# fdaPDE/fdaPDE-core

Measured on AMD Instinct MI355X. Metric: DOF/s assemble+solve, 3D P1 Laplacian; SpMV achieved HBM GB/s vs peak, higher is better.
Workload: dtype f64

## Files before the change

### fdapde-core_amd/capi.py

```python
from __future__ import annotations

import ctypes as C
import os

import numpy as np

_HERE = os.path.dirname(os.path.abspath(__file__))
LIB_PATH = os.environ.get("FDAPDE_HIP_LIB") or os.path.join(_HERE, "lib", "libfdapde_hip.so")

OK, EINVAL, ENOMEM, ENODEVICE, EHIP, ENOTINIT, ENOCONV, EUNSUPPORTED, ERCCL = range(9)
LAPLACIAN, DIFFUSION, ADVECTION, REACTION, DT = range(5)
SOLVER_AUTO, SOLVER_CG, SOLVER_BICGSTAB, SOLVER_CG_SR, SOLVER_CG_FUSED, SOLVER_GMRES, SOLVER_DENSE, SOLVER_PMG, SOLVER_AMG = range(9)
ASSEMBLY_ROWS, ASSEMBLY_ATOMIC, ASSEMBLY_COLOURED, ASSEMBLY_PARTITIONED, ASSEMBLY_WAVE = range(5)
MAT_STIFF, MAT_MASS = 0, 1


class Term(C.Structure):
    _fields_ = [("kind", C.c_int32), ("space_varying", C.c_int32), ("coef", C.c_double), ("cst", C.c_double * 9),
                ("data", C.POINTER(C.c_double))]


class Options(C.Structure):
    _fields_ = [("method", C.c_int32), ("maxit", C.c_int32), ("rtol", C.c_double), ("assembly", C.c_int32),
                ("check_every", C.c_int32), ("time_spmv", C.c_int32)]


class Info(C.Structure):
    _fields_ = [("iters", C.c_int32), ("converged", C.c_int32), ("relres", C.c_double), ("t_assemble_ms", C.c_double),
                ("t_solve_ms", C.c_double), ("t_setup_ms", C.c_double), ("spmv_avg_ms", C.c_double), ("spmv_timed", C.c_int32),
                ("method_used", C.c_int32), ("persistent", C.c_int32), ("gather_avg_ms", C.c_double), ("update_avg_ms", C.c_double),
                ("spmv_mean_ms", C.c_double), ("launch_ms", C.c_double)]


SYMBOLS = [
    "fdapde_abi_version", "fdapde_device_count", "fdapde_ctx_create", "fdapde_ctx_destroy", "fdapde_last_error",
    "fdapde_status_string", "fdapde_mesh_upload", "fdapde_dofs_build", "fdapde_dofs_get", "fdapde_dofs_set_boundary", "fdapde_sizes",
    "fdapde_pattern_get", "fdapde_quadrature_nodes", "fdapde_set_operator", "fdapde_set_forcing", "fdapde_set_dirichlet",
    "fdapde_init", "fdapde_assemble_operator", "fdapde_solver_prepare", "fdapde_solve", "fdapde_matrix_values", "fdapde_lump", "fdapde_force", "fdapde_solution",
    "fdapde_info_get", "fdapde_spmv", "fdapde_bench_spmv", "fdapde_tune", "fdapde_stream", "fdapde_synchronize",
    "fdapde_comm_unique_id", "fdapde_comm_init", "fdapde_halo_setup", "fdapde_solve_parabolic",
    "fdapde_lin_compute", "fdapde_lin_solve", "fdapde_eval_pointwise", "fdapde_cell_integrals", "fdapde_comm_init_callback", "fdapde_comm_set_exchange_callback", "fdapde_halo_setup_peers",
    "fdapde_solver_layout", "fdapde_topology_build", "fdapde_topology_get", "fdapde_comm_allreduce", "fdapde_comm_library", "fdapde_solver_layout_kind", "fdapde_solver_layout_partition", "fdapde_rowdist_setup", "fdapde_ctx_clone", "fdapde_comm_count",
    "fdapde_ctx_create_multi", "fdapde_ctx_devices", "fdapde_partition_build", "fdapde_partition_sizes", "fdapde_partition_get", "fdapde_partition_whole",
    "fdapde_partition_peers",
]
PARTITION_ROWDIST, PARTITION_ELEMENTS = 0, 1

_lib = None


def load() -> C.CDLL:
    global _lib
    if _lib is None:
        if not os.path.exists(LIB_PATH):
            raise ImportError(f"{LIB_PATH} is missing: build it with __graft_entry__.build() or `make -C fdapde-core_amd/csrc`. "
                              "There is no CPU fallback.")
        lib = C.CDLL(LIB_PATH)
        lib.fdapde_last_error.restype = C.c_char_p
        lib.fdapde_status_string.restype = C.c_char_p
        lib.fdapde_stream.restype = C.c_void_p
        lib.fdapde_comm_library.restype = C.c_char_p
        lib.fdapde_ctx_destroy.restype = None
        _lib = lib
    return _lib


class FdapdeError(RuntimeError):
    def __init__(self, status, msg):
        super().__init__(f"[status {status}] {msg}")
        self.status = status


def _dp(a):
    return a.ctypes.data_as(C.POINTER(C.c_double))


def _ip(a):
    return a.ctypes.data_as(C.POINTER(C.c_int32))


def _bp(a):
    return a.ctypes.data_as(C.POINTER(C.c_uint8))


class Operator:

    def __init__(self, terms=None):
        self.terms = list(terms or [])

    def __neg__(self):
        return Operator([(k, -c, cst, d) for (k, c, cst, d) in self.terms])

    def __add__(self, o):
        return Operator(self.terms + o.terms)

    def __sub__(self, o):
        return Operator(self.terms + (-o).terms)

    def __rmul__(self, s):
        return Operator([(k, float(s) * c, cst, d) for (k, c, cst, d) in self.terms])

    @property
    def is_symmetric(self):
        return all(k != ADVECTION for (k, _, _, _) in self.terms)

    def c_terms(self):
        arr = (Term * len(self.terms))()
        keep = []
        for t, (k, c, cst, d) in zip(arr, self.terms):
            t.kind, t.coef, t.space_varying = k, c, 0 if d is None else 1
            if cst is not None:
                for i, v in enumerate(np.asarray(cst, dtype=float).reshape(-1)):
                    t.cst[i] = v
            if d is not None:
                dd = np.ascontiguousarray(d, dtype=float)
                keep.append(dd)
                t.data = _dp(dd)
        return arr, keep


def laplacian():
    return Operator([(LAPLACIAN, 1.0, None, None)])


def diffusion(K):
    return Operator([(DIFFUSION, 1.0, np.asarray(K, dtype=float), None)])


def diffusion_field(Kq):
    return Operator([(DIFFUSION, 1.0, None, np.asarray(Kq, dtype=float))])


def advection(b):
    return Operator([(ADVECTION, 1.0, np.asarray(b, dtype=float), None)])


def advection_field(bq):
    return Operator([(ADVECTION, 1.0, None, np.asarray(bq, dtype=float))])


def reaction(c):
    return Operator([(REACTION, 1.0, np.asarray([c], dtype=float), None)])


def reaction_field(cq):
    return Operator([(REACTION, 1.0, None, np.asarray(cq, dtype=float))])


def dt():
    return Operator([(DT, 1.0, None, None)])


class Context:

    def __init__(self, device=0, devices=None):
        self.lib = load()
        self._ctx = C.c_void_p()
        if devices is not None:
            dv = (C.c_int32 * len(devices))(*[int(d) for d in devices])
            rc = self.lib.fdapde_ctx_create_multi(dv, len(devices), C.byref(self._ctx))
        else:
            rc = self.lib.fdapde_ctx_create(-1 if device is None else int(device), C.byref(self._ctx))
        if rc != OK:
            raise FdapdeError(rc, self.lib.fdapde_status_string(rc).decode())
        self.M = self.N = 0
        self.n_cells = self.n_nodes = 0

    def devices(self):
        n = C.c_int32()
        self._check(self.lib.fdapde_ctx_devices(self._ctx, C.byref(n), None, None, None, None))
        dv = (C.c_int32 * n.value)()
        form, tp, tr = C.c_int32(), C.c_double(), C.c_double()
        self._check(self.lib.fdapde_ctx_devices(self._ctx, C.byref(n), dv, C.byref(form), C.byref(tp), C.byref(tr)))
        return dict(devices=list(dv), form=form.value, t_partition_ms=tp.value, t_rank_setup_ms=tr.value)

    def partition_build(self, world, form=PARTITION_ROWDIST):
        self._check(self.lib.fdapde_partition_build(self._ctx, int(world), int(form)))
        self._part_world = int(world)

    def partition_get(self, rank):
        nn, nc = C.c_int64(), C.c_int64()
        self._check(self.lib.fdapde_partition_sizes(self._ctx, int(rank), C.byref(nn), C.byref(nc)))
        nn, nc = nn.value, nc.value
        nodes = np.zeros(nn * self.N)
        cells = np.zeros((nc, self.M + 1), dtype=np.int32)
        bnd = np.zeros(nn, dtype=np.uint8)
        l2g, cids, own = np.zeros(nn, dtype=np.int64), np.zeros(nc, dtype=np.int64), np.zeros(nn, dtype=np.int32)
        self._check(self.lib.fdapde_partition_get(self._ctx, int(rank), _dp(nodes), _ip(cells), _bp(bnd), l2g.ctypes.data_as(C.POINTER(C.c_int64)),
                                                  cids.ctypes.data_as(C.POINTER(C.c_int64)), _ip(own)))
        return dict(nodes=np.ascontiguousarray(nodes.reshape(self.N, nn).T), cells=cells, boundary=bnd, l2g=l2g, cell_ids=cids, owner=own)

    def partition_whole(self):
        part = np.zeros(self.n_cells, dtype=np.int32)
        own = np.zeros(self.n_nodes, dtype=np.int32)
        mask = np.zeros(self.n_nodes, dtype=np.uint64)
# ... 109 lines not shown
            self._check(self.lib.fdapde_set_forcing(self._ctx, None, 0))
            self._force_cols = 1
            return
        f = np.asarray(f_q, dtype=float)
        ncols = 1 if f.ndim == 1 else f.shape[1]
        self._force_cols = ncols
        flat = np.ascontiguousarray(f.reshape(f.shape[0], ncols).T).reshape(-1)
        self._check(self.lib.fdapde_set_forcing(self._ctx, _dp(flat), ncols))

    def set_dirichlet(self, g):
        if g is None:
            self._check(self.lib.fdapde_set_dirichlet(self._ctx, None))
        else:
            g = np.ascontiguousarray(g, dtype=float).reshape(-1)
            self._check(self.lib.fdapde_set_dirichlet(self._ctx, _dp(g)))

    def init(self, assembly=ASSEMBLY_ROWS):
        opt = Options(method=0, maxit=0, rtol=0.0, assembly=assembly, check_every=0, time_spmv=0)
        self._check(self.lib.fdapde_init(self._ctx, C.byref(opt)))

    def assemble_operator(self, which, op: Operator, assembly=ASSEMBLY_ROWS):
        terms, keep = op.c_terms()
        self._check(self.lib.fdapde_assemble_operator(self._ctx, which, len(op.terms), terms, assembly))

    def solver_prepare(self, with_dirichlet=True):
        self._check(self.lib.fdapde_solver_prepare(self._ctx, 1 if with_dirichlet else 0))

    def solve(self, method=SOLVER_AUTO, rtol=1e-10, maxit=0, check_every=0, raise_on_noconv=True, time_spmv=0):
        opt = Options(method=method, maxit=maxit, rtol=rtol, assembly=0, check_every=check_every, time_spmv=time_spmv)
        info = Info()
        rc = self.lib.fdapde_solve(self._ctx, C.byref(opt), C.byref(info))
        if rc != OK and (raise_on_noconv or rc != ENOCONV):
            self._check(rc)
        return info

    def solve_parabolic(self, times, initial_condition, dirichlet=None, method=SOLVER_AUTO, rtol=1e-10, maxit=0):
        times = np.asarray(times, dtype=float).reshape(-1)
        m, nd = times.size, self.sizes()["n_dofs"]
        u0 = np.ascontiguousarray(initial_condition, dtype=float).reshape(-1)
        g = None if dirichlet is None else np.ascontiguousarray(np.asarray(dirichlet, dtype=float).T).reshape(-1)
        out = np.zeros(nd * m)
        opt = Options(method=method, maxit=maxit, rtol=rtol, assembly=0, check_every=0, time_spmv=0)
        info = Info()
        self._check(self.lib.fdapde_solve_parabolic(self._ctx, C.byref(opt), int(m), C.c_double(times[1] - times[0]), _dp(u0),
                                                    None if g is None else _dp(g), _dp(out), C.byref(info)))
        return np.ascontiguousarray(out.reshape(m, nd).T), info

    def lin_compute(self, which=MAT_STIFF, values=None, symmetric=False):
        v = None if values is None else np.ascontiguousarray(values, dtype=float)
        self._check(self.lib.fdapde_lin_compute(self._ctx, which, None if v is None else _dp(v), 1 if symmetric else 0))

    def lin_solve(self, b, method=SOLVER_AUTO, rtol=1e-10, check_every=0, maxit=0):
        b = np.asarray(b, dtype=float)
        one = b.ndim == 1
        B = b.reshape(b.shape[0], -1)
        flat = np.ascontiguousarray(B.T).reshape(-1)
        out = np.zeros_like(flat)
        opt = Options(method=method, maxit=maxit, rtol=rtol, assembly=0, check_every=check_every, time_spmv=0)
        info = Info()
        self._check(self.lib.fdapde_lin_solve(self._ctx, C.byref(opt), _dp(flat), B.shape[1], _dp(out), C.byref(info)))
        X = np.ascontiguousarray(out.reshape(B.shape[1], B.shape[0]).T)
        return (X[:, 0] if one else X), info

    def eval_pointwise(self, locs):
        import scipy.sparse as sp

        locs = np.asarray(locs, dtype=float)
        if locs.ndim == 1:
            locs = locs.reshape(-1, 1)
        nl, s = locs.shape[0], self.sizes()
        flat = np.ascontiguousarray(locs.T).reshape(-1)
        cells = np.zeros(nl, dtype=np.int32)
        vals = np.zeros((nl, s["n_basis"]))
        self._check(self.lib.fdapde_eval_pointwise(self._ctx, C.c_int64(nl), _dp(flat), _ip(cells), _dp(vals)))
        dofs, _, _ = self.dofs_get()
        ok = cells >= 0
        rows = np.repeat(np.nonzero(ok)[0], s["n_basis"])
        cols = dofs[cells[ok]].reshape(-1)
        psi = sp.csr_matrix((vals[ok].reshape(-1), (rows, cols)), shape=(nl, s["n_dofs"]))
        return psi, np.ones(nl), cells

    def eval_areal(self, incidence):
        import scipy.sparse as sp

        inc = sp.csr_matrix(np.asarray(incidence) == 1, dtype=float)
        s = self.sizes()
        meas = np.zeros(self.n_cells)
        pint = np.zeros((self.n_cells, s["n_basis"]))
        self._check(self.lib.fdapde_cell_integrals(self._ctx, _dp(meas), _dp(pint)))
        dofs, _, _ = self.dofs_get()
        D = inc @ meas
        nb = s["n_basis"]
        cellmat = sp.csr_matrix((pint.reshape(-1), (np.repeat(np.arange(self.n_cells), nb), dofs.reshape(-1))),
                                shape=(self.n_cells, s["n_dofs"]))
        psi = sp.diags(1.0 / D) @ (inc @ cellmat)
        return psi.tocsr(), D

    def info(self):
        info = Info()
        self._check(self.lib.fdapde_info_get(self._ctx, C.byref(info)))
        return info

    def matrix_values(self, which=MAT_STIFF):
        out = np.zeros(self.sizes()["nnz"])
        self._check(self.lib.fdapde_matrix_values(self._ctx, which, _dp(out)))
        return out

    def lump(self, which=MAT_MASS):
        out = np.zeros(self.sizes()["n_dofs"])
        self._check(self.lib.fdapde_lump(self._ctx, which, _dp(out)))
        return out

    def force(self, ncols=None):
        have = getattr(self, "_force_cols", 1)
        if ncols is None:
            ncols = have
        if ncols < have:
            raise ValueError(f"force(): the context holds {have} forcing columns, a buffer for {ncols} was asked for")
        out = np.zeros(self.sizes()["n_dofs"] * ncols)
        self._check(self.lib.fdapde_force(self._ctx, _dp(out)))
        return out

    def solution(self):
        out = np.zeros(self.sizes()["n_dofs"])
        self._check(self.lib.fdapde_solution(self._ctx, _dp(out)))
        return out

    def spmv(self, which, x):
        x = np.ascontiguousarray(x, dtype=float)
        y = np.zeros_like(x)
        self._check(self.lib.fdapde_spmv(self._ctx, which, _dp(x), _dp(y)))
        return y

    def bench_spmv(self, reps=50):
        ms, by = C.c_double(), C.c_double()
        self._check(self.lib.fdapde_bench_spmv(self._ctx, reps, C.byref(ms), C.byref(by)))
        return ms.value, by.value

    def solver_layout(self, with_dirichlet=True):
        ni, nz, by = C.c_int64(), C.c_int64(), C.c_double()
        self._check(self.lib.fdapde_solver_layout(self._ctx, 1 if with_dirichlet else 0, C.byref(ni), C.byref(nz), C.byref(by)))
        return ni.value, nz.value, by.value

    def solver_layout_kind(self, with_dirichlet=True):
        k, sy, g, r = C.c_int32(), C.c_int32(), C.c_int32(), C.c_int32()
        self._check(self.lib.fdapde_solver_layout_kind(self._ctx, 1 if with_dirichlet else 0, C.byref(k), C.byref(sy), C.byref(g), C.byref(r)))
        return dict(kind=k.value, sym=sy.value, workgroups=g.value, rows_per_thread=r.value)

    def solver_layout_partition(self, with_dirichlet=True):
        p = C.c_int32()
        self._check(self.lib.fdapde_solver_layout_partition(self._ctx, 1 if with_dirichlet else 0, C.byref(p)))
        return p.value

    @staticmethod
    def comm_unique_id() -> bytes:
        buf = C.create_string_buffer(128)
        rc = load().fdapde_comm_unique_id(buf)
        if rc != OK:
            raise FdapdeError(rc, "fdapde_comm_unique_id failed (RCCL not loadable?)")
        return buf.raw

    def comm_init(self, world, rank, unique_id: bytes):
        self._check(self.lib.fdapde_comm_init(self._ctx, int(world), int(rank), C.c_char_p(unique_id)))

    def rowdist_setup(self, dof_key, dof_owner):
        k = np.ascontiguousarray(dof_key, dtype=np.int64)
        o = np.ascontiguousarray(dof_owner, dtype=np.int32)
        self._check(self.lib.fdapde_rowdist_setup(self._ctx, k.ctypes.data_as(C.POINTER(C.c_int64)), _ip(o)))

    def comm_allreduce(self, values, op="sum"):
        a = np.ascontiguousarray(np.asarray(values, dtype=float)).copy()
        self._check(self.lib.fdapde_comm_allreduce(self._ctx, _dp(a), int(a.size), 0 if op == "sum" else 1))
        return a

    def comm_count(self):
        n = C.c_int32(0)
        self._check(self.lib.fdapde_comm_count(self._ctx, C.byref(n)))
        return int(n.value)

    @staticmethod
    def comm_library():
        return (load().fdapde_comm_library() or b"").decode()

    def comm_init_callback(self, world, rank, allreduce):
        proto = C.CFUNCTYPE(C.c_int, C.c_void_p, C.POINTER(C.c_double), C.c_int64)

        def _cb(user, ptr, count):
            try:
                allreduce(np.ctypeslib.as_array(ptr, shape=(count,)))
                return 0
            except Exception:
                return 1

        self._ar_cb = proto(_cb)
        self._check(self.lib.fdapde_comm_init_callback(self._ctx, int(world), int(rank), self._ar_cb, None))

    def halo_setup(self, n_if_global, local_dof, if_index, owned):
        local_dof = np.ascontiguousarray(local_dof, dtype=np.int32)
        if_index = np.ascontiguousarray(if_index, dtype=np.int32)
        owned = np.ascontiguousarray(owned, dtype=np.uint8)
        self._check(self.lib.fdapde_halo_setup(self._ctx, C.c_int64(int(n_if_global)), C.c_int64(local_dof.size), _ip(local_dof),
                                               _ip(if_index), _bp(owned)))

    def comm_set_exchange_callback(self, exchange):
        proto = C.CFUNCTYPE(C.c_int, C.c_void_p, C.c_int32, C.POINTER(C.c_int32), C.POINTER(C.c_int64), C.POINTER(C.c_double), C.POINTER(C.c_double))

        def _cb(user, n_peers, ranks, offs, send, recv):
            try:
                off = np.ctypeslib.as_array(offs, shape=(n_peers + 1,))
                n = int(off[-1])
                exchange(np.ctypeslib.as_array(ranks, shape=(n_peers,)), off, np.ctypeslib.as_array(send, shape=(n,)),
                         np.ctypeslib.as_array(recv, shape=(n,)))
                return 0
            except Exception:
                return 1

        self._xchg_cb = proto(_cb)
        self._check(self.lib.fdapde_comm_set_exchange_callback(self._ctx, self._xchg_cb, None))

    def halo_setup_peers(self, peer_rank, peer_off, peer_dof, owned):
        peer_rank = np.ascontiguousarray(peer_rank, dtype=np.int32)
        peer_off = np.ascontiguousarray(peer_off, dtype=np.int64)
        peer_dof = np.ascontiguousarray(peer_dof, dtype=np.int32)
        owned = np.ascontiguousarray(owned, dtype=np.uint8)
        self._check(self.lib.fdapde_halo_setup_peers(self._ctx, C.c_int32(peer_rank.size), _ip(peer_rank),
                                                     peer_off.ctypes.data_as(C.POINTER(C.c_int64)), _ip(peer_dof), _bp(owned)))

    def tune(self, key, value):
        self._check(self.lib.fdapde_tune(self._ctx, key.encode(), int(value)))

    def stream(self):
        return self.lib.fdapde_stream(self._ctx)

    def synchronize(self):
        self._check(self.lib.fdapde_synchronize(self._ctx))
```

### fdapde-core_amd/csrc/capi.hip

```cpp
#include <algorithm>
#include <chrono>
#include <cmath>
#include <cstdio>
#include <cstdlib>
#include <cstring>
#include <new>

#include <dlfcn.h>
#include <hip/hip_ext.h>
#include <rccl/rccl.h>

#include "context.h"
#include "engine.h"

using namespace fdapde_engine;

extern "C" {

int fdapde_abi_version(void) { return FDAPDE_ABI_VERSION; }

int fdapde_device_count(void) {
    int n = 0;
    if (hipGetDeviceCount(&n) != hipSuccess) return 0;
    return n;
// ... 90 lines not shown
        if (c->h_sc) (void)hipHostFree(c->h_sc);
        (void)hipEventDestroy(c->ev0), (void)hipEventDestroy(c->ev1), (void)hipEventDestroy(c->ev_p0), (void)hipEventDestroy(c->ev_p1);
        for (hipEvent_t e : c->ev_spmv) (void)hipEventDestroy(e);
        (void)hipStreamDestroy(c->stream);
    }
    delete c->lin_state;
    delete c;
}

int fdapde_ctx_clone(const fdapde_ctx* src, fdapde_ctx** out) {
    if (!src || !out) return FDAPDE_EINVAL;
    *out = nullptr;
    if (src->group) return fdapde_engine::g_clone(src, out);
    fdapde_ctx* c = nullptr;
    if (int rc = fdapde_ctx_create(src->has_device ? src->device : -1, &c)) return rc;
    const int rc = fdapde_engine::e_ctx_clone(src, c);
    if (rc != FDAPDE_OK) {
        const_cast<fdapde_ctx*>(src)->err = "fdapde_ctx_clone: " + c->err;
        fdapde_ctx_destroy(c);
        return rc;
    }
    *out = c;
    return FDAPDE_OK;
}

const char* fdapde_last_error(const fdapde_ctx* c) { return c ? c->err.c_str() : "null context"; }

int fdapde_mesh_upload(fdapde_ctx* c, int M, int N, int64_t n_nodes, const double* nodes, int64_t n_cells,
                       const int32_t* cells, const uint8_t* bnd) {
    if (!c) return FDAPDE_EINVAL;
    if (c->group && M == 2 && N == 3)
        return fail(c, FDAPDE_EUNSUPPORTED, "fdapde_mesh_upload: a surface mesh (Triangulation<2,3>) takes a one-GPU context; the multi-device partitioner "
                                            "and its ranks are built for planar and volume meshes");
    if (c->group && M == 1)
        return fail(c, FDAPDE_EUNSUPPORTED, "fdapde_mesh_upload: a 1-D mesh (interval or linear network, Triangulation<1,N>) takes a one-GPU context; the "
                                            "multi-device partitioner and its ranks are built for planar and volume meshes");
    c->space_ready = c->dev_ready = c->colour_ready = c->fq_blk_ready = c->fq_bc_ready = c->stiff_stat_valid = false;
    c->assembled[0] = c->assembled[1] = c->force_ready = c->solved = c->dirichlet_applied = false;
    c->op.clear(), c->coef_of_op = false, c->fq_i.clear(), c->fq_cols = 0, c->g_i.clear(), c->have_g = false;
    if (c->topo_ready) dev_topology_release(&c->topo), c->topo_ready = false;
    c->mesh_on_dev = false;
    if (int rc = host_set_mesh(c->hs, M, N, n_nodes, nodes, n_cells, cells, bnd, c->err)) return rc;
    if (c->has_device) {
        const HostSpace& hs = c->hs;
        if (hipSetDevice(c->device) != hipSuccess || c->mesh_nodes.upload(hs.nodes.data(), hs.nodes.size(), c->stream) != hipSuccess ||
            c->mesh_cells.upload(hs.cells.data(), hs.cells.size(), c->stream) != hipSuccess ||
            c->mesh_nbnd.upload(hs.node_bnd.data(), hs.node_bnd.size(), c->stream) != hipSuccess || hipStreamSynchronize(c->stream) != hipSuccess) {
            c->mesh_nodes.release(), c->mesh_cells.release(), c->mesh_nbnd.release();
            c->err = "fdapde_mesh_upload: copying the mesh to the device failed";
            return FDAPDE_EHIP;
        }
        c->mesh_on_dev = true;
    }
    fdapde_engine::partition_free(c);
    if (c->group) fdapde_engine::g_mesh_changed(c);
    return FDAPDE_OK;
}

int fdapde_sizes(const fdapde_ctx* c, int64_t* n_dofs, int64_t* nnz, int32_t* n_basis, int32_t* n_quadrature, int64_t* n_edges) {
    if (!c || !c->space_ready) return FDAPDE_ENOTINIT;
    if (n_dofs) *n_dofs = c->hs.n_dofs;
    if (nnz) *nnz = c->hs.nnz;
    if (n_basis) *n_basis = c->hs.nb;
    if (n_quadrature) *n_quadrature = c->hs.nq;
    if (n_edges) *n_edges = c->hs.n_edges;
    return FDAPDE_OK;
}

int fdapde_dofs_build(fdapde_ctx* c, int order, int64_t* n_dofs) {
    if (!c) return FDAPDE_EINVAL;
    if (c->group) return fdapde_engine::g_dofs_build(c, order, n_dofs);
    return fdapde_engine::e_dofs_build(c, order, n_dofs);
}
int fdapde_topology_build(fdapde_ctx* c, int64_t* n_facets, int64_t* n_edges) {
    if (!c) return FDAPDE_EINVAL;
    return fdapde_engine::e_topology_build(c, n_facets, n_edges);
}
int fdapde_topology_get(fdapde_ctx* c, int32_t* neighbors, int32_t* cell_facets, int32_t* facet_nodes, int32_t* facet_cells, uint8_t* facet_boundary, int32_t* edge_nodes, uint8_t* edge_boundary, int32_t* face_edges) {
    if (!c) return FDAPDE_EINVAL;
    return fdapde_engine::e_topology_get(c, neighbors, cell_facets, facet_nodes, facet_cells, facet_boundary, edge_nodes, edge_boundary, face_edges);
}
int fdapde_dofs_set_boundary(fdapde_ctx* c, const uint8_t* bnd) {
    if (!c) return FDAPDE_EINVAL;
    if (c->group) return fdapde_engine::g_dofs_set_boundary(c, bnd);
    return fdapde_engine::e_dofs_set_boundary(c, bnd);
}
int fdapde_dofs_get(const fdapde_ctx* c, int32_t* dofs, uint8_t* bnd, double* coords) {
    if (!c) return FDAPDE_EINVAL;
    return fdapde_engine::e_dofs_get(c, dofs, bnd, coords);
}
int fdapde_pattern_get(const fdapde_ctx* c, int32_t* rowptr, int32_t* colidx) {
    if (!c) return FDAPDE_EINVAL;
    return fdapde_engine::e_pattern_get(c, rowptr, colidx);
}
int fdapde_quadrature_nodes(fdapde_ctx* c, double* out) {
    if (!c) return FDAPDE_EINVAL;
    return fdapde_engine::e_quadrature_nodes(c, out);
}
int fdapde_set_operator(fdapde_ctx* c, int32_t n_terms, const fdapde_term* terms) {
    if (!c) return FDAPDE_EINVAL;
    if (c->group) return fdapde_engine::g_set_operator(c, n_terms, terms);
    return fdapde_engine::e_set_operator(c, n_terms, terms);
}
int fdapde_set_forcing(fdapde_ctx* c, const double* f_q, int32_t n_cols) {
    if (!c) return FDAPDE_EINVAL;
    if (c->group) return fdapde_engine::g_set_forcing(c, f_q, n_cols);
    return fdapde_engine::e_set_forcing(c, f_q, n_cols);
}
int fdapde_set_dirichlet(fdapde_ctx* c, const double* g) {
    if (!c) return FDAPDE_EINVAL;
    if (c->group) return fdapde_engine::g_set_dirichlet(c, g);
    return fdapde_engine::e_set_dirichlet(c, g);
}
int fdapde_assemble_operator(fdapde_ctx* c, int32_t which, int32_t n_terms, const fdapde_term* terms, int32_t assembly) {
    if (!c) return FDAPDE_EINVAL;
    if (c->group) return fdapde_engine::g_assemble_operator(c, which, n_terms, terms, assembly);
    return fdapde_engine::e_assemble_operator(c, which, n_terms, terms, assembly);
}
int fdapde_init(fdapde_ctx* c, const fdapde_options* opt) {
    if (!c) return FDAPDE_EINVAL;
    if (c->group) return fdapde_engine::g_init(c, opt);
    return fdapde_engine::e_init(c, opt);
}
int fdapde_eval_pointwise(fdapde_ctx* c, int64_t n_locs, const double* locs_colmajor, int32_t* cell_ids, double* values) {
    if (!c) return FDAPDE_EINVAL;
    return fdapde_engine::e_eval_pointwise(c, n_locs, locs_colmajor, cell_ids, values);
}
int fdapde_cell_integrals(fdapde_ctx* c, double* measure, double* psi_int) {
    if (!c) return FDAPDE_EINVAL;
    return fdapde_engine::e_cell_integrals(c, measure, psi_int);
}
int fdapde_solver_prepare(fdapde_ctx* c, int32_t with_dirichlet) {
    if (!c) return FDAPDE_EINVAL;
    if (c->group) return fdapde_engine::g_solver_prepare(c, with_dirichlet);
    return fdapde_engine::e_solver_prepare(c, with_dirichlet);
}
int fdapde_solver_layout(fdapde_ctx* c, int32_t with_dirichlet, int64_t* n_interior, int64_t* nnz_interior, double* streamed_bytes) {
    if (!c) return FDAPDE_EINVAL;
    if (c->group) return fdapde_engine::g_layout_kind(c, with_dirichlet, nullptr, nullptr, nullptr, nullptr);
    return fdapde_engine::e_solver_layout(c, with_dirichlet, n_interior, nnz_interior, streamed_bytes);
}
int fdapde_solver_layout_kind(fdapde_ctx* c, int32_t with_dirichlet, int32_t* kind, int32_t* symmetric_storage, int32_t* workgroups, int32_t* rows_per_thread) {
    if (!c) return FDAPDE_EINVAL;
    if (c->group) return fdapde_engine::g_layout_kind(c, with_dirichlet, kind, symmetric_storage, workgroups, rows_per_thread);
    return fdapde_engine::e_solver_layout_kind(c, with_dirichlet, kind, symmetric_storage, workgroups, rows_per_thread);
}
int fdapde_solver_layout_partition(fdapde_ctx* c, int32_t with_dirichlet, int32_t* partition) {
    int32_t kind = 0;
    if (int rc = fdapde_solver_layout_kind(c, with_dirichlet, &kind, nullptr, nullptr, nullptr)) return rc;
    const fdapde_ctx::Persist& ps = c->ps[with_dirichlet ? 1 : 0];
    if (partition) *partition = (kind == 2 || kind == 3) && ps.ok ? (ps.meta.bisect ? 1 : 0) : -1;
    return FDAPDE_OK;
}
int fdapde_solve(fdapde_ctx* c, const fdapde_options* opt, fdapde_info* info) {
    if (!c) return FDAPDE_EINVAL;
    if (c->group && opt && opt->method == FDAPDE_SOLVER_AMG) return fdapde_engine::fail(c, FDAPDE_EUNSUPPORTED, "FDAPDE_SOLVER_AMG takes one-GPU contexts, not a multi-device context");
    if (c->group) return fdapde_engine::g_solve(c, opt, info);
    return fdapde_engine::e_solve(c, opt, info);
}
int fdapde_solve_parabolic(fdapde_ctx* c, const fdapde_options* opt, int32_t n_times, double delta_t, const double* initial_condition, const double* dirichlet, double* solution, fdapde_info* info) {
    if (!c) return FDAPDE_EINVAL;
    if (c->group && opt && opt->method == FDAPDE_SOLVER_AMG) return fdapde_engine::fail(c, FDAPDE_EUNSUPPORTED, "FDAPDE_SOLVER_AMG takes one-GPU contexts, not a multi-device context");
    if (c->group) return fdapde_engine::g_solve_parabolic(c, opt, n_times, delta_t, initial_condition, dirichlet, solution, info);
    return fdapde_engine::e_solve_parabolic(c, opt, n_times, delta_t, initial_condition, dirichlet, solution, info);
}
int fdapde_lin_compute(fdapde_ctx* c, int32_t which, const double* values, int32_t symmetric) {
    if (!c) return FDAPDE_EINVAL;
    if (c->group) return fdapde_engine::g_lin_compute(c, which, values, symmetric);
    return fdapde_engine::e_lin_compute(c, which, values, symmetric);
}
int fdapde_lin_solve(fdapde_ctx* c, const fdapde_options* opt, const double* b, int32_t n_rhs, double* x, fdapde_info* info) {
    if (!c) return FDAPDE_EINVAL;
    if (c->group && opt && opt->method == FDAPDE_SOLVER_AMG) return fdapde_engine::fail(c, FDAPDE_EUNSUPPORTED, "FDAPDE_SOLVER_AMG takes one-GPU contexts, not a multi-device context");
    if (c->group) return fdapde_engine::g_lin_solve(c, opt, b, n_rhs, x, info);
    return fdapde_engine::e_lin_solve(c, opt, b, n_rhs, x, info);
}
int fdapde_matrix_values(fdapde_ctx* c, int32_t which, double* values) {
    if (!c) return FDAPDE_EINVAL;
    if (c->group) return fdapde_engine::g_matrix_values(c, which, values);
    return fdapde_engine::e_matrix_values(c, which, values);
}
int fdapde_lump(fdapde_ctx* c, int32_t which, double* diag) {
    if (!c) return FDAPDE_EINVAL;
    if (c->group) return fdapde_engine::g_lump(c, which, diag);
    return fdapde_engine::e_lump(c, which, diag);
}
int fdapde_force(fdapde_ctx* c, double* force) {
    if (!c) return FDAPDE_EINVAL;
    if (c->group) return fdapde_engine::g_force(c, force);
    return fdapde_engine::e_force(c, force);
}
int fdapde_solution(fdapde_ctx* c, double* solution) {
    if (!c) return FDAPDE_EINVAL;
    if (c->group) return fdapde_engine::g_solution(c, solution);
    return fdapde_engine::e_solution(c, solution);
}
int fdapde_spmv(fdapde_ctx* c, int32_t which, const double* x, double* y) {
    if (!c) return FDAPDE_EINVAL;
    if (c->group) return fdapde_engine::g_spmv(c, which, x, y);
    return fdapde_engine::e_spmv(c, which, x, y);
}
int fdapde_bench_spmv(fdapde_ctx* c, int32_t reps, double* avg_ms, double* algorithmic_bytes) {
    if (!c) return FDAPDE_EINVAL;
    if (c->group) return fail(c, FDAPDE_EUNSUPPORTED, "fdapde_bench_spmv: a multi-device context wires its own ranks");
    return fdapde_engine::e_bench_spmv(c, reps, avg_ms, algorithmic_bytes);
}
int fdapde_comm_unique_id(void* out128) {
    return fdapde_engine::e_comm_unique_id(out128);
}
int fdapde_comm_init(fdapde_ctx* c, int32_t world, int32_t rank, const void* unique_id128) {
    if (!c) return FDAPDE_EINVAL;
    if (c->group) return fail(c, FDAPDE_EUNSUPPORTED, "fdapde_comm_init: a multi-device context wires its own ranks");
    return fdapde_engine::e_comm_init(c, world, rank, unique_id128);
}
int fdapde_comm_allreduce(fdapde_ctx* c, double* host_inout, int32_t n, int32_t op) {
    if (!c) return FDAPDE_EINVAL;
    if (c->group) return fail(c, FDAPDE_EUNSUPPORTED, "fdapde_comm_allreduce: a multi-device context wires its own ranks");
    return fdapde_engine::e_comm_allreduce(c, host_inout, n, op);
}
int fdapde_comm_count(fdapde_ctx* c, int32_t* ranks) {
    if (!c) return FDAPDE_EINVAL;
    return fdapde_engine::e_comm_count(c, ranks);
}
int fdapde_comm_init_callback(fdapde_ctx* c, int32_t world, int32_t rank, fdapde_allreduce_fn fn, void* user) {
    if (!c) return FDAPDE_EINVAL;
    if (c->group) return fail(c, FDAPDE_EUNSUPPORTED, "fdapde_comm_init_callback: a multi-device context wires its own ranks");
    return fdapde_engine::e_comm_init_callback(c, world, rank, fn, user);
}
int fdapde_halo_setup(fdapde_ctx* c, int64_t n_if_global, int64_t n_if_local, const int32_t* local_dof, const int32_t* if_index, const uint8_t* owned) {
    if (!c) return FDAPDE_EINVAL;
    if (c->group) return fail(c, FDAPDE_EUNSUPPORTED, "fdapde_halo_setup: a multi-device context wires its own ranks");
    return fdapde_engine::e_halo_setup(c, n_if_global, n_if_local, local_dof, if_index, owned);
}
int fdapde_rowdist_setup(fdapde_ctx* c, const int64_t* dof_key, const int32_t* dof_owner) {
    if (!c) return FDAPDE_EINVAL;
    if (c->group) return fail(c, FDAPDE_EUNSUPPORTED, "fdapde_rowdist_setup: a multi-device context wires its own ranks");
    return fdapde_engine::e_rowdist_setup(c, dof_key, dof_owner);
}
int fdapde_comm_set_exchange_callback(fdapde_ctx* c, fdapde_exchange_fn fn, void* user) {
    if (!c) return FDAPDE_EINVAL;
    if (c->group) return fail(c, FDAPDE_EUNSUPPORTED, "fdapde_comm_set_exchange_callback: a multi-device context wires its own ranks");
    return fdapde_engine::e_comm_set_exchange_callback(c, fn, user);
}
int fdapde_halo_setup_peers(fdapde_ctx* c, int32_t n_peers, const int32_t* peer_rank, const int64_t* peer_off, const int32_t* peer_dof, const uint8_t* owned) {
    if (!c) return FDAPDE_EINVAL;
    if (c->group) return fail(c, FDAPDE_EUNSUPPORTED, "fdapde_halo_setup_peers: a multi-device context wires its own ranks");
    return fdapde_engine::e_halo_setup_peers(c, n_peers, peer_rank, peer_off, peer_dof, owned);
}

int fdapde_ctx_create_multi(const int32_t* devices, int32_t n_devices, fdapde_ctx** out) {
    return fdapde_engine::g_create(devices, n_devices, out);
}
int fdapde_ctx_devices(const fdapde_ctx* c, int32_t* n_devices, int32_t* devices, int32_t* form, double* t_partition_ms, double* t_rank_setup_ms) {
    if (!c) return FDAPDE_EINVAL;
    return fdapde_engine::g_info(c, n_devices, devices, form, t_partition_ms, t_rank_setup_ms);
}
int fdapde_partition_build(fdapde_ctx* c, int32_t world, int32_t form) {
    if (!c) return FDAPDE_EINVAL;
    if (c->group) return fail(c, FDAPDE_EUNSUPPORTED, "fdapde_partition_build: a multi-device context partitions its mesh itself (fdapde_dofs_build)");
    return fdapde_engine::e_partition_build(c, world, form);
}
int fdapde_partition_sizes(const fdapde_ctx* c, int32_t rank, int64_t* n_nodes, int64_t* n_cells) {
    if (!c) return FDAPDE_EINVAL;
    return fdapde_engine::e_partition_sizes(c, rank, n_nodes, n_cells);
}
int fdapde_partition_get(fdapde_ctx* c, int32_t rank, double* nodes_colmajor, int32_t* cells, uint8_t* boundary, int64_t* node_ids, int64_t* cell_ids, int32_t* node_owner) {
    if (!c) return FDAPDE_EINVAL;
    return fdapde_engine::e_partition_get(c, rank, nodes_colmajor, cells, boundary, node_ids, cell_ids, node_owner);
}
int fdapde_partition_whole(fdapde_ctx* c, int32_t* cell_rank, int32_t* node_owner, uint64_t* node_ranks) {
    if (!c) return FDAPDE_EINVAL;
    return fdapde_engine::e_partition_whole(c, cell_rank, node_owner, node_ranks);
}
int fdapde_partition_peers(fdapde_ctx* c, int32_t rank, int32_t* n_peers, int32_t* peer_rank, int64_t* peer_off, int32_t* peer_node, uint8_t* owned, int64_t* n_shared) {
    if (!c) return FDAPDE_EINVAL;
    return fdapde_engine::e_partition_peers(c, rank, n_peers, peer_rank, peer_off, peer_node, owned, n_shared);
}

int fdapde_info_get(const fdapde_ctx* c, fdapde_info* info) {
    if (!c || !info) return FDAPDE_EINVAL;
    *info = c->info;
    return FDAPDE_OK;
}

const char* fdapde_comm_library(void) { return g_rccl.path.c_str(); }

int fdapde_tune(fdapde_ctx* c, const char* key, int32_t value) {
    if (!c || !key) return FDAPDE_EINVAL;
    if (!c->dev_ready) return fail(c, FDAPDE_ENOTINIT, "call fdapde_dofs_build first");
    if (c->group) return fdapde_engine::g_tune(c, key, value);
    const std::string k(key);
    drop_graph(c);
    if (k == "spmv_variant" && value >= 0 && value <= 2) c->spmv_variant = value;
    else if (k == "spmv_team" && (value == 2 || value == 4 || value == 8 || value == 16 || value == 32 || value == 64)) {
        if (value != c->spmv_team) c->sp_built[0] = c->sp_built[1] = false, c->sp_cur = -1, c->solved = false, c->scaled_owner = fdapde_ctx::kScaledNone;
        c->spmv_team = value;
    }
    else if (k == "spmv_unroll" && value >= 1 && value <= 8) c->spmv_unroll = value;
    else if (k == "spmv_ablate") c->spmv_ablate = value;
    else if (k == "spmv_c16" && (value == 0 || value == 1)) c->spmv_c16 = value;
    else if (k == "spmv_deep" && (value == 0 || value == 1)) c->spmv_deep = value;
    else if (k == "cgf_split" && (value == 0 || value == 1)) c->cgf_split = value;
    else if (k == "cgf_v" && (value == 1 || value == 2 || value == 4 || value == 8)) c->cgf_v = value;
    else if (k == "use_graph" && (value == 0 || value == 1)) c->use_graph = value;
    else if (k == "cgf_band" && (value == 0 || value == 1)) c->cgf_band = value;
    else if (k == "cgf_nt" && value >= 0 && value <= 15) c->cgf_nt = value;
    else if (k == "cgf_lazy" && (value == 0 || value == 1)) c->cgf_lazy = value;
    else if (k == "multi_rhs" && (value == 0 || value == 1)) c->multi_rhs = value;
    else if (k == "asm_fq_block" && (value == 0 || value == 1)) c->asm_fq_block = value;
    else if (k == "asm_fuse_mass" && value >= 0 && value <= 3) c->asm_fuse_mass = value;
    else if (k == "asm_items" && (value == 0 || value == 1)) c->asm_items = value;
    else if (k == "asm_items_fuse" && (value == 0 || value == 1)) c->asm_items_fuse = value;
    else if (k == "bicg_restart" && (value == 0 || value == 1)) c->bicg_restart = value;
    else if (k == "bicg_shadow" && value >= 0 && value <= 2) c->bicg_shadow = value;
    else if (k == "gmres_m" && value >= 2 && value <= 200) c->gmres_m = value;
    else if (k == "persist_exp_lds" && (value == 0 || value == 1)) {
        c->persist_exp_lds = value;
        c->ps[0].tried = c->ps[0].ok = c->ps[1].tried = c->ps[1].ok = false, c->scaled_owner = fdapde_ctx::kScaledNone;
        fdapde_engine::drop_graph(c);
    }
    else if (k == "dense_rows" && value >= 0 && value <= 8192) c->dense_rows = value, c->lin_dense.ready = false, c->lin_dense.failed = false;
    else if (k == "dense_after" && value >= 0) c->dense_after = value;
    else if (k == "dense_block" && (value == 0 || value == 1)) c->dense_block = value;
    else if (k == "dense_direct" && (value == 0 || value == 1)) c->dense_direct = value;
    else if (k == "dense_fold" && (value == 0 || value == 1)) c->dense_fold = value;
    else if (k == "dense_multi" && (value == 0 || value == 1)) c->dense_multi = value;
    else if (k == "pmg_inner_tol_exp" && value >= 1 && value <= 12) c->pmg_inner_rtol = std::pow(10.0, -(double)value);
    else if (k == "pmg_inner_maxit" && value >= 1) c->pmg_inner_maxit = value;
    else if (k == "pmg_auto" && (value == 0 || value == 1)) c->pmg_auto = value;
    else if (k == "pmg_blocked" && (value == 0 || value == 1)) c->pmg_blocked = value;
    else if (k == "pmg_smooth" && (value == 0 || value == 1)) c->pmg_smooth = value;
    else if (k == "pmg_setup_check" && (value == 0 || value == 1)) c->pmg_setup_check = value;
    else if (k == "amg_coarse_rows" && value >= 1 && value <= 8192) c->amg_coarse_rows = value;
    else if (k == "amg_setup_check" && (value == 0 || value == 1)) c->amg_setup_check = value;
    else if (k == "pmg_restart" && value >= 2 && value <= 50) c->pmg_restart = (int)value;
    else if (k == "pmg_outer" && (value == 0 || value == 1)) c->pmg_outer = value;
    else if (k == "pmg_auto_rows" && value >= 0) c->pmg_auto_rows = value;
    else if (k == "pmg_auto_first_rows" && value >= 0) c->pmg_auto_first_rows = value;
    else if (k == "dense_bulk" && (value == 0 || value == 1)) c->dense_bulk = value;
    else if (k == "dense_hostb" && (value == 0 || value == 1)) c->dense_hostb = value;
    else if (k == "small_rows" && value >= 0) c->small_rows = value;
    else if (k == "small_front_rows" && value >= 0) c->small_front_rows = value;
    else if (k == "auto_gmres" && (value == 0 || value == 1)) c->auto_gmres = value;
    else if (k == "asm_split_varying" && (value == 0 || value == 1)) c->asm_split_varying = value;
    else if (k == "asm_row_stat" && (value == 0 || value == 1)) c->asm_row_stat = value, c->stiff_stat_valid = false;
    else if (k == "asm_fq_bc" && (value == 0 || value == 1)) c->asm_fq_bc = value, c->fq_bc_ready = c->fq_bc_ready && value;
    else if (k == "persist" && (value == 0 || value == 1)) c->persist = value, c->persist_broken = false;
    else if (k == "persist_time" && (value == 0 || value == 1)) c->persist_time = value;
    else if (k == "persist_coop" && (value == 0 || value == 1)) c->persist_coop = value;
    else if (k == "persist_bicg" && (value == 0 || value == 1)) c->persist_bicg = value;
    else if (k == "persist_fill_fused" && (value == 0 || value == 1)) c->persist_fill_fused = value;
    else if (k == "persist_prefetch" && (value == 0 || value == 1)) c->persist_prefetch = value;
    else if (k == "persist_cols" && (value == 0 || value == 1)) c->persist_cols = value;
    else if (k == "persist_direct" && (value == 0 || value == 1)) c->persist_direct = value;
    else if (k == "persist_wide_gj" && (value == 4 || value == 6 || value == 12)) {
        c->persist_wide_gj = value;
        for (auto& ps : c->ps) ps.attr_set = nullptr;
    }
    else if ((k == "persist_wide" && (value == 0 || value == 1)) || (k == "persist_max_wg" && value >= 0)) {
        if (k == "persist_wide") c->persist_wide = value;
        else c->persist_max_wg = value;
        for (auto& ps : c->ps) ps.tried = ps.ok = ps.filled = false;
    }
    else if (k == "persist_direct_spin_us" && value >= 0 && value <= 1000000) c->persist_direct_spin_us = value;
    else if (k == "persist_single_rows" && value >= 0 && value <= 8192) {
        c->persist_single_rows = value;
        for (auto& ps : c->ps) ps.tried = ps.ok = ps.filled = false;
    }
    else if (k == "persist_partition" && value >= 0 && value <= 2) {
        c->persist_partition = value;
        for (auto& ps : c->ps) ps.tried = ps.ok = ps.filled = false;
    }
    else if (k == "persist_late" && (value == 0 || value == 1)) {
        c->persist_late = value;
        for (auto& ps : c->ps) ps.tried = ps.ok = ps.filled = false;
    }
    else if (k == "rowdist_max_wg" && value >= 0) {
        c->rd.max_wg = value;
        for (auto& L : c->rd.lay) L.tried = L.ok = false;
    } else if (k == "rowdist_share" && value >= 1) {
        c->rd.max_wg = std::max(1, c->n_cu / value);
        for (auto& L : c->rd.lay) L.tried = L.ok = false;
    } else if (k == "rowdist_timeout_first_ms" && value >= 1) c->rd.timeout_first_ms = value;
    else if (k == "rowdist_flat_gather" && value >= -1 && value <= 1) c->rd.flat_gather = value;
    else if (k == "persist_timeout_us" && value >= 100 && value <= 10000000) c->persist_timeout_us = value;
    else if (k == "persist_debug_stall" && value >= 0) c->persist_debug_stall = value;
    else if (k == "persist_retry" && value == 1) c->persist_broken = false, c->persist_retry_in = 0, c->persist_backoff = 8;
    else if (k == "blocked" && value >= 0 && value <= 2) c->blocked = value;
    else if (k == "persist_gather_waves" && (value == 1 || value == 4)) c->persist_gather_waves = value;
    else if (k == "persist_poll_sleep" && value >= 0 && value <= 3) c->persist_poll_sleep = value;
    else if (k == "persist_balance" && (value == 0 || value == 1)) {
        c->persist_balance = value;
        for (auto& ps : c->ps) ps.tried = ps.ok = ps.filled = false;
    } else if (k == "persist_sym" && value >= 0 && value <= 2) {
        c->persist_sym = value;
        for (auto& ps : c->ps) ps.tried = ps.ok = ps.filled = false;
    }
    else if (k == "spmv_ntv" && value >= -1 && value <= 1) c->spmv_ntv = value;
    else if (k == "spmv_bpx" && value >= 1 && value <= 1024) {
        c->spmv_grid = 8 * value;
        HIPCHK(c, hipSetDevice(c->device));
        HIPCHK(c, hipStreamSynchronize(c->stream));
        HIPCHK(c, c->part_a.alloc(2 * (size_t)c->spmv_grid));
    } else return fail(c, FDAPDE_EINVAL, "unknown tuning key or value out of range");
    return FDAPDE_OK;
}

void* fdapde_stream(fdapde_ctx* c) { return c ? (void*)c->stream : nullptr; }

int fdapde_synchronize(fdapde_ctx* c) {
    if (!c) return FDAPDE_EINVAL;
    if (int rc = need_device(c)) return rc;
    if (c->group)
        if (int rc = fdapde_engine::g_synchronize(c)) return rc;
    HIPCHK(c, hipSetDevice(c->device));
    HIPCHK(c, hipStreamSynchronize(c->stream));
    HIPCHK(c, hipDeviceSynchronize());
    return FDAPDE_OK;
}

}
```

### fdapde-core_amd/csrc/context.h

```cpp
#ifndef FDAPDE_CONTEXT_H
#define FDAPDE_CONTEXT_H

#include <cstdint>
#include <memory>
#include <functional>
#include <string>
#include <vector>

#include <dlfcn.h>
#include <hip/hip_ext.h>
#include <hip/hip_runtime.h>
#include <rccl/rccl.h>

#include "../../include/fdapde_hip.h"
#include "dev_persist.h"
#include "dev_setup.h"
#include "dev_topology.h"
#include "internal.h"

namespace fdapde_engine {
struct Group;
struct AmgHierarchy;
}
namespace fdapde_hip {
// ... 207 lines not shown
    int persist_direct_spin_us = 2000;
    int32_t* h_ctl = nullptr;
    double* h_sc = nullptr;
    int spmv_grid = 0, rb_per_band = 0, vec_grid = 0, n_rb = 0, cg_grid = 0;
    int spmv_variant = 2;
    int spmv_team = 16, spmv_unroll = 4, spmv_ablate = 0;
    int lds_limit = 96 * 1024;
    DBuf<int32_t> sp_rowptr[2], sp_colidx[2], sp_map[2], sp_tbase[2], sp_vrow[2];
    int64_t sp_nv[2] = {0, 0};
    int sval_layout = -2;
    DBuf<uint16_t> sp_col16[2];
    int64_t sp_wide[2] = {0, 0};
    int spmv_ntv = -1;
    int sp_team = 0;
    int spmv_c16 = 1;
    int use_graph = 0;
    hipGraphExec_t cg_graph_exec = nullptr;
    GraphKey cg_graph_key{};
    int cgf_lazy = 1;
    int cgf_nt = 7;
    int cgf_band = 1;
    int cgf_split = 0;
    int cgf_v = 8;
    int spmv_deep = 0;
    int64_t sp_nnz[2] = {0, 0};
    bool sp_built[2] = {false, false};
    int sp_cur = -1;
    bool sval_stale = false;
    const double* sval_A = nullptr;
    int persist_fill_fused = 0;
    enum { kScaledNone = 0, kScaledSolve, kScaledParabolic, kScaledLin, kScaledPmg };
    int scaled_owner = kScaledNone;
    ncclComm_t comm = nullptr;
    fdapde_allreduce_fn ar_fn = nullptr;
    void* ar_user = nullptr;
    std::vector<double> ar_host;
    DBuf<double> ar_dev;
    int world = 1, rank = 0;
    bool halo_ready = false;
    int64_t n_if = 0, n_loc_if = 0;
    DBuf<int32_t> halo_dof, halo_pos;
    DBuf<int32_t> halo_inv, if_slot;
    DBuf<uint8_t> owned;
    DBuf<double> hbuf, sbuf;
    bool peer_mode = false;
    fdapde_exchange_fn xchg_fn = nullptr;
    void* xchg_user = nullptr;
    std::vector<int32_t> peer_rank;
    std::vector<int64_t> peer_off;
    DBuf<int32_t> peer_send_dof;
    DBuf<int32_t> peer_src_off, peer_src;
    DBuf<double> peer_sendbuf, peer_recvbuf;
    std::vector<double> xchg_send_h, xchg_recv_h;
    struct PeerDirect {
        bool on = false;
        int (*arrive)(void*) = nullptr;
        void* user = nullptr;
        int parity = 0, ar_parity = 0;
        int64_t n_send = 0;
        DBuf<const double*> remote[2];
        DBuf<double> slots;
        DBuf<const double*> slot_ptr;
    } xd;
    static constexpr int kSlotDoubles = 64;
    DBuf<double> lin_mat;
    bool lin_ready = false, lin_symmetric = false;
    DBuf<double> lin_sq;
    bool lin_sq_ready = false;
    int multi_rhs = 1;
    SolveStateHolder* lin_state = nullptr;
    int n_cu = 0;
    int persist = 1;
    int persist_time = 1;
    int persist_balance = 1;
    int persist_sym = 2;
    int persist_gather_waves = 4, persist_poll_sleep = 2;
    bool persist_broken = false;
    int persist_retry_in = 0, persist_backoff = 8;
    struct Persist {
        bool tried = false, ok = false;
        PersistLayout meta;
        int32_t lds_cap = 0, imp_cap = 0;
        size_t lds_bytes = 0;
        DBuf<int32_t> slot_dof, sl_off, ell_src, exp_off, imp_off, imp_pos;
        DBuf<int32_t> ell_col;
        bool stream = false;
        bool exp_lds = false;
        DBuf<int64_t> ell_off;
        DBuf<uint16_t> ell_code, exp_slot;
        DBuf<double> ell_val;
        DBuf<unsigned long long> amax;
        DBuf<uint8_t> wg_late;
        DBuf<unsigned long long> board;
        DBuf<unsigned long long> board_cols;
        int per_cu = 0;
        bool filled = false;
        uint32_t epoch_next = 0;
        const void* attr_set = nullptr;
        bool built_plain = false;
    } ps[2];
    struct RowDist {
        bool ready = false;
        std::vector<int32_t> owner_i;
        std::vector<int64_t> key_i;
        DBuf<uint8_t> owned;
        int max_wg = 0;
        int flat_gather = -1;
        int timeout_first_ms = 2000;
        struct Layout {
            bool tried = false, ok = false;
            Persist ps;
            int32_t n_ghost = 0, G_tot = 0, g_base = 0;
            DBuf<int32_t> rexp_off, rexp_peer, rexp_pos;
            DBuf<uint16_t> rexp_slot;
            DBuf<uint8_t> wg_late;
            DBuf<unsigned long long> rboard;
            DBuf<unsigned long long*> peer_pboard, peer_dboard;
            std::vector<void*> ipc_opened;
            std::vector<int32_t> x_rank;
            std::vector<int64_t> x_soff, x_roff;
            DBuf<int32_t> x_send_dof, x_recv_dof;
            DBuf<double> x_sendbuf, x_recvbuf;
        } lay[2];
    } rd;
    DBuf<double> persist_stats;
    DBuf<double> persist_x;
    DBuf<double> persist_xs;
    int persist_wide_gj = 12;
    int persist_wide = 1;
    int persist_max_wg = 0;
    double persist_launch_ms = 0;
    int persist_host_below = 32768;
    int persist_cols = 1;
    DBuf<double> cols_b, cols_r, cols_x, cols_sc, cols_part;
    DBuf<int32_t> cols_ctl;
    struct EvalGrid {
        bool ready = false;
        DBuf<int32_t> ptr, cells, dims;
        DBuf<double> lo, invh;
        void release() { ptr.release(), cells.release(), dims.release(), lo.release(), invh.release(), ready = false; }
    } eval_grid;
    DBuf<double> eval_locs, eval_vals;
    DBuf<int32_t> eval_out;
    std::function<int()> persist_tail;
    int h_ctl_seen = 4;
    bool ev1_at_end = false;
    int64_t small_rows = 8192;
    int64_t small_front_rows = 2048;
    bool front_used = false;
    bool tail_in_launch = false;
    bool defer_end_sync = false;
    int persist_single_rows = 2048;
    int persist_prefetch = 1;
    int persist_partition = 2;
    int persist_late = 0;
    int persist_plain = 0;
    int persist_bicg = 1;
    int persist_coop = 0;
    int persist_timeout_us = 5000;
    int persist_debug_stall = 0;
    struct Blocked {
        bool tried = false, ok = false, filled = false;
        PersistLayout meta;
        int32_t imp_cap = 0;
        size_t lds_bytes = 0;
        DBuf<int32_t> slot_dof, sl_off, ell_src, imp_off, imp_dof, drop_dof;
        DBuf<int64_t> ell_off;
        DBuf<uint16_t> ell_code;
        DBuf<double> ell_val;
    } bk[2];
    int bk_cur = -1;
    int blocked = 1;
    DevTopology topo;
    bool topo_ready = false;
    bool part_ready = false, wave_ready = false;
    int32_t part_colours = 0;
    int64_t n_parts = 0;
    DBuf<int32_t> part_cells, part_off, part_slots, wave_slots;
    DBuf<uint8_t> part_shared;
    std::vector<double> persist_host_stats;
    struct Pmg {
        fdapde_ctx* coarse = nullptr;
        bool ready = false;
        int64_t init_seen = -1;
        double extra_seen = 0.0;
        DBuf<int32_t> pa, pb;
        DBuf<int32_t> fine_cell;
        DBuf<int32_t> rt_ptr, rt_idx;
        DBuf<double> rt_w, dinv, vec, part, dots, basis;
        int np = 1;
        double setup_ms = 0;
        int last_coarse_iters = 0, last_coarse_calls = 0;
        DBuf<int32_t> flag;
        const double* fine_A = nullptr;
        int64_t fine_key = -1;
        int fine_bnd = -1;
        double omega = 0.0;
        const double* omega_A = nullptr;
        int64_t omega_key = -1;
        int omega_bnd = -1;
        double omega_extra = 0.0;
        SolveState coarse_ss;
    } pmg;
    fdapde_engine::AmgHierarchy* amg = nullptr;
    fdapde_engine::AmgHierarchy* amg_lin = nullptr;
    int64_t amg_lin_epoch = 0;
    int64_t amg_coarse_rows = 1024;
    int amg_setup_check = 0;
    int64_t init_count = 0;
    bool matrix_dirty = true;
    bool last_init_rows = false;
    double pmg_inner_rtol = 1e-1;
    int pmg_inner_maxit = 200;
    int pmg_auto = 1;
    int pmg_outer = 0;
    int pmg_setup_check = 0;
    int pmg_restart = 50;
    int pmg_smooth = 1;
    int64_t pmg_auto_first_rows = 1000000;
    int64_t open_solves = 0;
    int pmg_blocked = 1;
    int64_t pmg_auto_rows = 300000;
    struct Dense {
        DBuf<double> X;
        int64_t n = 0;
        int use_bnd = 0;
        const double* A = nullptr;
        const int32_t *rowptr = nullptr, *colidx = nullptr;
        const uint8_t* bnd = nullptr;
        bool ready = false, refine = false, failed = false;
        double check = 0, build_ms = 0;
    } lin_dense, step_dense, solve_dense;
    int dense_bulk = 1;
    int dense_fold = 1;
    int dense_hostb = 0;
    int dense_direct = 0;
    int dense_multi = 1;
    int dense_block = 1;
    int dense_rows = 8192;
    int dense_after = 2;
    int64_t lin_cols = 0;
    double lin_krylov_ms = 0;
    DBuf<double> dn_b, dn_x, dn_r, dn_e;
    DBuf<unsigned int> dn_cnt;
    fdapde_engine::Group* group = nullptr;
    fdapde_hip::DevPartition* partition = nullptr;
    double partition_ms = 0;
    std::vector<uint64_t> partition_mask_h;
};

#endif
```

### fdapde-core_amd/csrc/dev_persist.h

```cpp
#ifndef FDAPDE_DEV_PERSIST_H
#define FDAPDE_DEV_PERSIST_H

#include <cstdint>
#include <string>
#include <vector>

#include "internal.h"

namespace fdapde_hip {

struct DevPersist {
    int32_t *slot_dof = nullptr, *sl_off = nullptr, *ell_src = nullptr, *exp_off = nullptr, *imp_off = nullptr, *imp_pos = nullptr;
    int64_t* ell_off = nullptr;
    uint16_t *ell_code = nullptr, *exp_slot = nullptr;
    int32_t* drop_dof = nullptr;
};
void dev_persist_release(DevPersist* p);
int dev_build_persist_layout(int64_t nd, int32_t max_row, const int32_t* d_rowptr, const int32_t* d_colidx, const uint8_t* d_bnd, bool use_bnd,
                             int n_wg, int lds_entries, int blocked_rows, const int32_t* block_rows, int sym_mode, bool balance, void* stream, PersistLayout& pl, DevPersist* out,
                             std::string& err);

int dev_build_persist_layout_bisect(int64_t nd, int32_t max_row, const int32_t* d_rowptr, const int32_t* d_colidx, const uint8_t* d_bnd, bool use_bnd, int M,
                                    int N, const double* d_coords, const int32_t* d_i2e, int G, int lds_entries, int sym_mode, void* stream, PersistLayout& pl,
                                    DevPersist* out, std::vector<int32_t>* perm_out, std::vector<int32_t>* rows_out, std::string& err);

void dev_persist_preload();
}
#endif
```

### fdapde-core_amd/csrc/dev_persist.hip

```cpp
#include <hip/hip_runtime.h>
#include <hipcub/hipcub.hpp>

#include <algorithm>
#include <chrono>
#include <cstdint>
#include <string>
#include <vector>

#include "dev_persist.h"

namespace fdapde_hip {

namespace {

#define DP_CHK(expr)                                                          \
    do {                                                                      \
        hipError_t e__ = (expr);                                              \
        if (e__ != hipSuccess) {                                              \
            err = std::string(#expr) + ": " + hipGetErrorString(e__);         \
            return FDAPDE_EHIP;                                               \
        }                                                                     \
    } while (0)

struct Arena {
// ... 638 lines not shown
    DP_CHK(hipMemcpyAsync(o.exp_off, h_exp_off.data(), sizeof(int32_t) * ((size_t)G + 1), hipMemcpyHostToDevice, st));
    DP_CHK(hipMemcpyAsync(o.imp_off, h_imp_off.data(), sizeof(int32_t) * ((size_t)G + 1), hipMemcpyHostToDevice, st));
    phase("boards");
    const int64_t n_sl = (int64_t)G * nsl;
    Tmp<int32_t> pairs, pscan, max_block;
    DP_CHK(pairs.alloc((size_t)n_sl + 1));
    DP_CHK(pscan.alloc((size_t)n_sl + 1));
    DP_CHK(max_block.alloc(1));
    DP_CHK(hipMemsetAsync(pairs.p + n_sl, 0, sizeof(int32_t), st));
    DP_CHK(hipMemsetAsync(max_block.p, 0, sizeof(int32_t), st));
    hipLaunchKernelGGL(k_slice_pairs, dim3(grid_of(n_sl)), dim3(256), 0, st, n_sl, o.slot_dof, len.p, pairs.p);
    if (int rc = exclusive_sum(sc, pairs.p, pscan.p, n_sl + 1, st, err)) return rc;
    DP_CHK(hipMalloc(reinterpret_cast<void**>(&o.sl_off), sizeof(int32_t) * (size_t)G * (nsl + 1)));
    DP_CHK(hipMalloc(reinterpret_cast<void**>(&o.ell_off), sizeof(int64_t) * ((size_t)G + 1)));
    hipLaunchKernelGGL(k_slice_offsets, dim3(grid_of((int64_t)G * (nsl + 1))), dim3(256), 0, st, G, nsl, pscan.p, o.sl_off, o.ell_off, max_block.p);
    int32_t h_total = 0, h_maxb = 0;
    DP_CHK(hipMemcpyAsync(&h_total, pscan.p + n_sl, sizeof(int32_t), hipMemcpyDeviceToHost, st));
    DP_CHK(hipMemcpyAsync(&h_maxb, max_block.p, sizeof(int32_t), hipMemcpyDeviceToHost, st));
    DP_CHK(hipStreamSynchronize(st));
    pl.n_entries = (int64_t)h_total * 128;
    pl.max_block = (int64_t)h_maxb * 128;
    const size_t n_alloc = (size_t)pl.n_entries + 256;
    DP_CHK(hipMalloc(reinterpret_cast<void**>(&o.ell_code), sizeof(uint16_t) * n_alloc));
    DP_CHK(hipMalloc(reinterpret_cast<void**>(&o.ell_src), sizeof(int32_t) * n_alloc));
    DP_CHK(hipMemsetAsync(o.ell_code, 0, sizeof(uint16_t) * n_alloc, st));
    DP_CHK(hipMemsetAsync(o.ell_src, 0xff, sizeof(int32_t) * n_alloc, st));
    hipLaunchKernelGGL(k_fill_ell, dim3(grid_of((int64_t)G * S)), dim3(256), 0, st, (int64_t)G * S, (int32_t)S, nsl, o.slot_dof, d_rowptr, d_colidx, keep.p, wg.p,
                       slot_of.p, blocked ? (const int32_t*)nullptr : board_of.p, o.imp_off, o.imp_pos, o.sl_off, o.ell_off, sym ? 1 : 0, sym ? own.p : (const int32_t*)nullptr, o.ell_code, o.ell_src);
    DP_CHK(hipGetLastError());
    DP_CHK(hipStreamSynchronize(st));
    phase("sliced ELL");
    guard.armed = false;
    *out = o;
    return FDAPDE_OK;
}

namespace {

__global__ void k_bis_rows(int64_t nd, int64_t n_int, int N, const uint8_t* keep, const int32_t* irow_scan, const int32_t* len, const int32_t* i2e,
                           const double* coords, const double* bb , double span, int32_t* cost, uint32_t* q, int32_t* ord) {
    const int64_t d = (int64_t)blockIdx.x * blockDim.x + threadIdx.x;
    if (d >= nd || !keep[d]) return;
    const int64_t i = irow_scan[d], e = i2e ? i2e[d] : d;
    cost[i] = len[d] + 2, ord[i] = (int32_t)i;
    for (int a = 0; a < 3; ++a) {
        uint32_t v = 0;
        if (a < N) {
            const double lo = bb[a], hi = bb[3 + a];
            const double w = hi > lo ? (coords[(int64_t)a * nd + e] - lo) / (hi - lo) : 0.0;
            v = (uint32_t)llround(fmin(1.0, fmax(0.0, w)) * span);
        }
        q[(int64_t)a * n_int + i] = v;
    }
}
constexpr int kBisPer = 16;
__global__ __launch_bounds__(256) void k_bis_extent(int64_t n_int, const int32_t* ord, const int32_t* segb, int nseg, const uint32_t* q, uint32_t* ext_lo, uint32_t* ext_hi) {
    const int64_t base = (int64_t)blockIdx.x * (256 * kBisPer);
    int32_t cur = -1;
    uint32_t lo[3] = {0xffffffffu, 0xffffffffu, 0xffffffffu}, hi[3] = {0u, 0u, 0u};
    for (int it = 0; it < kBisPer; ++it) {
        const int64_t p = base + (int64_t)it * 256 + threadIdx.x;
        if (p >= n_int) break;
        const int32_t seg = wg_of_irow(segb, nseg, p);
        if (seg != cur) {
            if (cur >= 0)
                for (int a = 0; a < 3; ++a) atomicMin(&ext_lo[cur * 3 + a], lo[a]), atomicMax(&ext_hi[cur * 3 + a], hi[a]);
            cur = seg;
            for (int a = 0; a < 3; ++a) lo[a] = 0xffffffffu, hi[a] = 0u;
        }
        const int64_t row = ord[p];
        for (int a = 0; a < 3; ++a) {
            const uint32_t v = q[(int64_t)a * n_int + row];
            lo[a] = min(lo[a], v), hi[a] = max(hi[a], v);
        }
    }
    const int32_t c0 = __shfl(cur, 0);
    const bool one = __ballot(cur != c0) == 0ull;
    if (one) {
        for (int a = 0; a < 3; ++a)
            for (int o = 32; o >= 1; o >>= 1) lo[a] = min(lo[a], (uint32_t)__shfl_xor((int)lo[a], o)), hi[a] = max(hi[a], (uint32_t)__shfl_xor((int)hi[a], o));
        if ((threadIdx.x & 63) != 0) cur = -1;
    }
    if (cur >= 0)
        for (int a = 0; a < 3; ++a) atomicMin(&ext_lo[cur * 3 + a], lo[a]), atomicMax(&ext_hi[cur * 3 + a], hi[a]);
}
__global__ void k_bis_keys(int64_t n_int, const int32_t* ord, const int32_t* segb, const int32_t* segg, int nseg, const uint32_t* q, const uint32_t* ext_lo,
                           const uint32_t* ext_hi, uint64_t* key) {
    const int64_t p = (int64_t)blockIdx.x * blockDim.x + threadIdx.x;
    if (p >= n_int) return;
    const int32_t seg = wg_of_irow(segb, nseg, p);
    uint64_t c = 0;
    if (segg[seg] > 1) {
        int axis = 0;
        uint32_t best = 0;
        for (int a = 0; a < 3; ++a) {
            const uint32_t ext = ext_hi[seg * 3 + a] - ext_lo[seg * 3 + a];
            if (ext > best) best = ext, axis = a;
        }
        c = q[(int64_t)axis * n_int + ord[p]];
    }
    key[p] = ((uint64_t)(uint32_t)seg << 31) | c;
}
__global__ void k_bis_gather_cost(int64_t n_int, const int32_t* ord, const int32_t* cost, int64_t* out) {
    const int64_t p = (int64_t)blockIdx.x * blockDim.x + threadIdx.x;
    if (p <= n_int) out[p] = p < n_int ? cost[ord[p]] : 0;
}
__global__ __launch_bounds__(512) void k_bis_split(int nseg, const int32_t* segb, const int32_t* segg, const int64_t* pre, int32_t* nb, int32_t* ng) {
    __shared__ int32_t sg[512];
    const int s = threadIdx.x;
    if (s < nseg) sg[s] = segg[s];
    __syncthreads();
    if (s >= nseg) return;
    int off = 0;
    for (int t = 0; t < s; ++t) off += sg[t] > 1 ? 2 : 1;
    const int32_t b = segb[s], e = segb[s + 1], g = sg[s];
    if (s == 0) nb[0] = 0;
    if (g == 1) {
        nb[off + 1] = e, ng[off] = 1;
        return;
    }
    const int32_t gl = g / 2, gr = g - gl;
    const int64_t share = (pre[e] - pre[b]) * gl / g;
    int32_t lo = b, hi = e;
    while (lo < hi) {
        const int32_t mid = (lo + hi) >> 1;
        if (pre[mid] - pre[b] >= share) hi = mid; else lo = mid + 1;
    }
    const int32_t split = max(b + gl, min(e - gr, lo));
    nb[off + 1] = split, ng[off] = gl, nb[off + 2] = e, ng[off + 1] = gr;
}
__global__ void k_bis_numbering(int64_t nd, int64_t n_int, const uint8_t* keep, const int32_t* irow_scan, const int32_t* pos_of_row, const int32_t* rowptr,
                                int32_t* new_of_old, int32_t* old_of_new, int32_t* len_new) {
    const int64_t d = (int64_t)blockIdx.x * blockDim.x + threadIdx.x;
    if (d >= nd) return;
    const int64_t np = keep[d] ? pos_of_row[irow_scan[d]] : n_int + (d - irow_scan[d]);
    new_of_old[d] = (int32_t)np, old_of_new[np] = (int32_t)d, len_new[np] = rowptr[d + 1] - rowptr[d];
}
__global__ void k_bis_invert(int64_t n, const int32_t* p, int32_t* inv) {
    const int64_t i = (int64_t)blockIdx.x * blockDim.x + threadIdx.x;
    if (i < n) inv[p[i]] = (int32_t)i;
}
__global__ void k_bis_entries(int64_t nd, const int32_t* rowptr, const int32_t* colidx, const int32_t* new_of_old, const int32_t* rowptr_new, uint64_t* key,
                              int32_t* val) {
    const int64_t d = (int64_t)blockIdx.x * blockDim.x + threadIdx.x;
    if (d >= nd) return;
    const int32_t np = new_of_old[d];
    int64_t at = rowptr_new[np];
    for (int32_t k = rowptr[d]; k < rowptr[d + 1]; ++k, ++at) key[at] = ((uint64_t)(uint32_t)np << 32) | (uint32_t)new_of_old[colidx[k]], val[at] = k;
}
__global__ void k_bis_map_back(int64_t n, const int32_t* map, int32_t* v) {
    const int64_t i = (int64_t)blockIdx.x * blockDim.x + threadIdx.x;
    if (i < n && v[i] >= 0) v[i] = map[v[i]];
}
inline int bits_for(int64_t n) {
    int b = 1;
    while ((int64_t(1) << b) < n) ++b;
    return b;
}

}

int dev_build_persist_layout_bisect(int64_t nd, int32_t max_row, const int32_t* d_rowptr, const int32_t* d_colidx, const uint8_t* d_bnd, bool use_bnd, int M,
                                    int N, const double* d_coords, const int32_t* d_i2e, int G, int lds_entries, int sym_mode, void* stream, PersistLayout& pl,
                                    DevPersist* out, std::vector<int32_t>* perm_out, std::vector<int32_t>* rows_out, std::string& err) {
    hipStream_t st = static_cast<hipStream_t>(stream);
    if (G < 2 || G > kPersistT || nd < 1 || max_row > 255 || N < 1 || N > 3) return FDAPDE_EUNSUPPORTED;
    Arena arena;
    ArenaScope arena_scope(&arena);
    Scratch sc;
    Tmp<uint8_t> keep;
    Tmp<int32_t> keep32, irow_scan, len;
    DP_CHK(keep.alloc((size_t)nd));
    DP_CHK(keep32.alloc((size_t)nd + 1));
    DP_CHK(irow_scan.alloc((size_t)nd + 1));
    DP_CHK(len.alloc((size_t)nd));
    DP_CHK(hipMemsetAsync(keep32.p + nd, 0, sizeof(int32_t), st));
    hipLaunchKernelGGL(k_keep_flags, dim3(grid_of(nd)), dim3(256), 0, st, nd, d_bnd, use_bnd ? 1 : 0, keep.p, keep32.p);
    if (int rc = exclusive_sum(sc, keep32.p, irow_scan.p, nd + 1, st, err)) return rc;
    hipLaunchKernelGGL(k_row_lengths, dim3(grid_of(nd)), dim3(256), 0, st, nd, d_rowptr, d_colidx, keep.p, len.p);
    int32_t h_nint = 0, h_nnz = 0;
    DP_CHK(hipMemcpyAsync(&h_nint, irow_scan.p + nd, sizeof(int32_t), hipMemcpyDeviceToHost, st));
    DP_CHK(hipMemcpyAsync(&h_nnz, d_rowptr + nd, sizeof(int32_t), hipMemcpyDeviceToHost, st));
    DP_CHK(hipStreamSynchronize(st));
    const int64_t n_int = h_nint, nnz = h_nnz;
    if (n_int < (int64_t)G) return FDAPDE_EUNSUPPORTED;
    Tmp<double> bb;
    DP_CHK(bb.alloc(6));
    for (int a = 0; a < N; ++a) {
        size_t need = 0;
        DP_CHK(hipcub::DeviceReduce::Min(nullptr, need, d_coords + (int64_t)a * nd, bb.p + a, (int)nd, st));
        DP_CHK(sc.need(need));
        DP_CHK(hipcub::DeviceReduce::Min(sc.p, need, d_coords + (int64_t)a * nd, bb.p + a, (int)nd, st));
        DP_CHK(hipcub::DeviceReduce::Max(sc.p, need, d_coords + (int64_t)a * nd, bb.p + 3 + a, (int)nd, st));
    }
    Tmp<int32_t> cost, ord_a, ord_b, seg_a, seg_b, sgg_a, sgg_b;
    Tmp<uint32_t> q, ext;
    Tmp<uint64_t> key_a, key_b;
    Tmp<int64_t> c2, pre;
    DP_CHK(cost.alloc((size_t)n_int));
    DP_CHK(ord_a.alloc((size_t)n_int));
    DP_CHK(ord_b.alloc((size_t)n_int));
    DP_CHK(q.alloc(3 * (size_t)n_int));
    DP_CHK(key_a.alloc((size_t)n_int));
    DP_CHK(key_b.alloc((size_t)n_int));
    DP_CHK(c2.alloc((size_t)n_int + 1));
    DP_CHK(pre.alloc((size_t)n_int + 1));
    DP_CHK(seg_a.alloc((size_t)G + 1));
    DP_CHK(seg_b.alloc((size_t)G + 1));
    DP_CHK(sgg_a.alloc((size_t)G));
    DP_CHK(sgg_b.alloc((size_t)G));
    DP_CHK(ext.alloc(6 * (size_t)G));
    const double span = persist_bisect_span(M, N, nd);
    hipLaunchKernelGGL(k_bis_rows, dim3(grid_of(nd)), dim3(256), 0, st, nd, n_int, N, keep.p, irow_scan.p, len.p, d_i2e, d_coords, bb.p, span, cost.p, q.p, ord_a.p);
    std::vector<int32_t> segg{G};
    {
        const int32_t b0[2] = {0, (int32_t)n_int};
        DP_CHK(hipMemcpyAsync(seg_a.p, b0, sizeof(b0), hipMemcpyHostToDevice, st));
        DP_CHK(hipMemcpyAsync(sgg_a.p, segg.data(), sizeof(int32_t), hipMemcpyHostToDevice, st));
        DP_CHK(hipStreamSynchronize(st));
    }
    int32_t *ord = ord_a.p, *ord_n = ord_b.p, *segb = seg_a.p, *segb_n = seg_b.p, *sgg = sgg_a.p, *sgg_n = sgg_b.p;
    while (*std::max_element(segg.begin(), segg.end()) > 1) {
        const int nseg = (int)segg.size();
        DP_CHK(hipMemsetAsync(ext.p, 0xff, sizeof(uint32_t) * 3 * (size_t)nseg, st));
        DP_CHK(hipMemsetAsync(ext.p + 3 * (size_t)G, 0, sizeof(uint32_t) * 3 * (size_t)nseg, st));
        hipLaunchKernelGGL(k_bis_extent, dim3((unsigned)((n_int + 256 * kBisPer - 1) / (256 * kBisPer))), dim3(256), 0, st, n_int, ord, segb, nseg, q.p, ext.p, ext.p + 3 * (size_t)G);
        hipLaunchKernelGGL(k_bis_keys, dim3(grid_of(n_int)), dim3(256), 0, st, n_int, ord, segb, sgg, nseg, q.p, ext.p, ext.p + 3 * (size_t)G, key_a.p);
        if (int rc = sort_pairs(sc, key_a.p, key_b.p, ord, ord_n, n_int, 31 + bits_for(nseg), st, err)) return rc;
        hipLaunchKernelGGL(k_bis_gather_cost, dim3(grid_of(n_int + 1)), dim3(256), 0, st, n_int, ord_n, cost.p, c2.p);
        if (int rc = exclusive_sum(sc, c2.p, pre.p, n_int + 1, st, err)) return rc;
        hipLaunchKernelGGL(k_bis_split, dim3(1), dim3(512), 0, st, nseg, segb, sgg, pre.p, segb_n, sgg_n);
        std::swap(ord, ord_n), std::swap(segb, segb_n), std::swap(sgg, sgg_n);
        std::vector<int32_t> ng;
        for (int32_t g : segg) {
            if (g > 1) ng.push_back(g / 2), ng.push_back(g - g / 2);
            else ng.push_back(1);
        }
        segg.swap(ng);
    }
    DP_CHK(hipGetLastError());
    std::vector<int32_t> h_b((size_t)G + 1), h_rows((size_t)G);
    DP_CHK(hipMemcpyAsync(h_b.data(), segb, sizeof(int32_t) * ((size_t)G + 1), hipMemcpyDeviceToHost, st));
    DP_CHK(hipStreamSynchronize(st));
    for (int g = 0; g < G; ++g) {
        h_rows[(size_t)g] = h_b[(size_t)g + 1] - h_b[(size_t)g];
        if (h_rows[(size_t)g] < 1) return FDAPDE_EUNSUPPORTED;
    }
    if (perm_out) {
        perm_out->resize((size_t)n_int);
        DP_CHK(hipMemcpyAsync(perm_out->data(), ord, sizeof(int32_t) * (size_t)n_int, hipMemcpyDeviceToHost, st));
        DP_CHK(hipStreamSynchronize(st));
    }
    Tmp<int32_t> pos_of_row, new_of_old, old_of_new, len_new, rowptr_new, colidx_new, src_a, src_new;
    Tmp<uint8_t> bnd_new;
    Tmp<uint64_t> ek_a, ek_b;
    DP_CHK(pos_of_row.alloc((size_t)n_int));
    DP_CHK(new_of_old.alloc((size_t)nd));
    DP_CHK(old_of_new.alloc((size_t)nd));
    DP_CHK(len_new.alloc((size_t)nd + 1));
    DP_CHK(rowptr_new.alloc((size_t)nd + 1));
    DP_CHK(colidx_new.alloc((size_t)nnz + 2));
    DP_CHK(src_a.alloc((size_t)nnz));
    DP_CHK(src_new.alloc((size_t)nnz));
    DP_CHK(ek_a.alloc((size_t)nnz));
    DP_CHK(ek_b.alloc((size_t)nnz));
    DP_CHK(bnd_new.alloc((size_t)nd));
    hipLaunchKernelGGL(k_bis_invert, dim3(grid_of(n_int)), dim3(256), 0, st, n_int, ord, pos_of_row.p);
    DP_CHK(hipMemsetAsync(len_new.p + nd, 0, sizeof(int32_t), st));
    hipLaunchKernelGGL(k_bis_numbering, dim3(grid_of(nd)), dim3(256), 0, st, nd, n_int, keep.p, irow_scan.p, pos_of_row.p, d_rowptr, new_of_old.p, old_of_new.p,
                       len_new.p);
    if (int rc = exclusive_sum(sc, len_new.p, rowptr_new.p, nd + 1, st, err)) return rc;
    hipLaunchKernelGGL(k_bis_entries, dim3(grid_of(nd)), dim3(256), 0, st, nd, d_rowptr, d_colidx, new_of_old.p, rowptr_new.p, ek_a.p, src_a.p);
    if (nnz > 0) {
        if (int rc = sort_pairs(sc, ek_a.p, ek_b.p, src_a.p, src_new.p, nnz, 32 + bits_for(nd), st, err)) return rc;
        hipLaunchKernelGGL(k_low32, dim3(grid_of(nnz)), dim3(256), 0, st, nnz, ek_b.p, colidx_new.p);
    }
    DP_CHK(hipMemsetAsync(colidx_new.p + nnz, 0, 2 * sizeof(int32_t), st));
    DP_CHK(hipMemsetAsync(bnd_new.p, 0, (size_t)n_int, st));
    if (nd > n_int) DP_CHK(hipMemsetAsync(bnd_new.p + n_int, 1, (size_t)(nd - n_int), st));
    DP_CHK(hipGetLastError());
    DevPersist o;
    if (int rc = dev_build_persist_layout(nd, max_row, rowptr_new.p, colidx_new.p, bnd_new.p, true, G, lds_entries, 0, h_rows.data(), sym_mode, false, stream, pl, &o,
                                          err))
        return rc;
    const int64_t n_slots = (int64_t)pl.G * pl.R * kPersistT, n_ent = pl.n_entries + 256;
    hipLaunchKernelGGL(k_bis_map_back, dim3(grid_of(n_slots)), dim3(256), 0, st, n_slots, old_of_new.p, o.slot_dof);
    hipLaunchKernelGGL(k_bis_map_back, dim3(grid_of(n_ent)), dim3(256), 0, st, n_ent, src_new.p, o.ell_src);
    if (hipGetLastError() != hipSuccess || hipStreamSynchronize(st) != hipSuccess) {
        dev_persist_release(&o);
        err = "bisection layout: mapping back failed";
        return FDAPDE_EHIP;
    }
    if (rows_out) *rows_out = std::move(h_rows);
    *out = o;
    return FDAPDE_OK;
}

void dev_persist_preload() {
    hipFuncAttributes attr;
    (void)hipFuncGetAttributes(&attr, reinterpret_cast<const void*>(&k_keep_flags));
    (void)hipGetLastError();
}

}
```

### fdapde-core_amd/csrc/host_bisect.cpp

```cpp
#include <algorithm>
#include <cmath>
#include <cstdint>
#include <numeric>
#include <vector>

#include "internal.h"

namespace fdapde_hip {

void host_bisect_quantise(int N, int64_t n, const double* pts_colmajor, const int32_t* i2e, double span, std::vector<uint32_t>& q) {
    q.assign((size_t)3 * (size_t)n, 0u);
    if (n < 1) return;
    for (int d = 0; d < N && d < 3; ++d) {
        const double* x = pts_colmajor + (int64_t)d * n;
        double lo = x[0], hi = x[0];
        for (int64_t i = 1; i < n; ++i) lo = std::min(lo, x[i]), hi = std::max(hi, x[i]);
        for (int64_t i = 0; i < n; ++i) {
            const double p = x[i2e ? i2e[(size_t)i] : i];
            const double w = hi > lo ? (p - lo) / (hi - lo) : 0.0;
            q[(size_t)d * (size_t)n + (size_t)i] = (uint32_t)std::llround(std::min(1.0, std::max(0.0, w)) * span);
        }
    }
}

int host_bisect_partition(int64_t n_int, const int32_t* cost, const uint32_t* qx, const uint32_t* qy, const uint32_t* qz, int G, std::vector<int32_t>& perm,
                          std::vector<int32_t>& block_rows) {
    if (G < 1 || n_int < (int64_t)G) return FDAPDE_EUNSUPPORTED;
    const uint32_t* q[3] = {qx, qy, qz};
    perm.resize((size_t)n_int);
    std::iota(perm.begin(), perm.end(), 0);
    std::vector<int32_t> segb{0, (int32_t)n_int}, segg{G};
    std::vector<int64_t> pre;
    while (*std::max_element(segg.begin(), segg.end()) > 1) {
        std::vector<int32_t> nb{0}, ng;
        for (size_t s = 0; s < segg.size(); ++s) {
            const int32_t b = segb[s], e = segb[s + 1], g = segg[s];
            if (g == 1) {
                nb.push_back(e), ng.push_back(1);
                continue;
            }
            int axis = 0;
            uint32_t best = 0;
            for (int d = 0; d < 3; ++d) {
                uint32_t lo = 0xffffffffu, hi = 0;
                for (int32_t p = b; p < e; ++p) lo = std::min(lo, q[d][(size_t)perm[(size_t)p]]), hi = std::max(hi, q[d][(size_t)perm[(size_t)p]]);
                if (hi - lo > best) best = hi - lo, axis = d;
            }
            const uint32_t* qa = q[axis];
            std::stable_sort(perm.begin() + b, perm.begin() + e, [qa](int32_t a, int32_t c) { return qa[(size_t)a] < qa[(size_t)c]; });
            pre.resize((size_t)(e - b) + 1);
            pre[0] = 0;
            for (int32_t p = b; p < e; ++p) pre[(size_t)(p - b) + 1] = pre[(size_t)(p - b)] + cost[(size_t)perm[(size_t)p]];
            const int32_t gl = g / 2, gr = g - gl;
            const int64_t share = pre[(size_t)(e - b)] * gl / g;
            int32_t split = b + (int32_t)(std::lower_bound(pre.begin(), pre.begin() + (e - b), share) - pre.begin());
            split = std::max(b + gl, std::min(e - gr, split));
            nb.push_back(split), ng.push_back(gl), nb.push_back(e), ng.push_back(gr);
        }
        segb.swap(nb), segg.swap(ng);
    }
    block_rows.resize((size_t)G);
    for (int g = 0; g < G; ++g) block_rows[(size_t)g] = segb[(size_t)g + 1] - segb[(size_t)g];
    return FDAPDE_OK;
}

int host_build_persist_layout_bisect(const HostSpace& hs, bool use_bnd, int G, int lds_entries, PersistLayout& pl, int sym_mode, const uint32_t* q,
                                     std::vector<int32_t>* perm_out, std::vector<int32_t>* rows_out) {
    const int64_t nd = hs.n_dofs;
    auto dropped = [&](int64_t d) { return use_bnd && hs.dof_bnd_i[(size_t)d] != 0; };
    std::vector<int32_t> irow_dof, cost;
    std::vector<uint32_t> qi[3];
    for (int64_t d = 0; d < nd; ++d) {
        if (dropped(d)) continue;
        int32_t len = 0;
        for (int32_t k = hs.rowptr_i[(size_t)d]; k < hs.rowptr_i[(size_t)d + 1]; ++k) {
            const int32_t c = hs.colidx_i[(size_t)k];
            len += c != d && !dropped(c);
        }
        irow_dof.push_back((int32_t)d), cost.push_back(len + 2);
        for (int a = 0; a < 3; ++a) qi[a].push_back(q[(size_t)a * (size_t)nd + (size_t)d]);
    }
    const int64_t n_int = (int64_t)irow_dof.size();
    std::vector<int32_t> perm, rows;
    if (int rc = host_bisect_partition(n_int, cost.data(), qi[0].data(), qi[1].data(), qi[2].data(), G, perm, rows)) return rc;
    std::vector<int32_t> old_of_new((size_t)nd), new_of_old((size_t)nd);
    for (int64_t p = 0; p < n_int; ++p) old_of_new[(size_t)p] = irow_dof[(size_t)perm[(size_t)p]];
    {
        int64_t p = n_int;
        for (int64_t d = 0; d < nd; ++d)
            if (dropped(d)) old_of_new[(size_t)p++] = (int32_t)d;
    }
    for (int64_t p = 0; p < nd; ++p) new_of_old[(size_t)old_of_new[(size_t)p]] = (int32_t)p;
    HostSpace hp;
    hp.n_dofs = nd, hp.nnz = hs.nnz, hp.max_row = hs.max_row;
    hp.dof_bnd_i.assign((size_t)nd, 0);
    for (int64_t p = n_int; p < nd; ++p) hp.dof_bnd_i[(size_t)p] = 1;
    hp.rowptr_i.resize((size_t)nd + 1);
    hp.colidx_i.resize((size_t)hs.nnz + 2);
    hp.colidx_i[(size_t)hs.nnz] = hp.colidx_i[(size_t)hs.nnz + 1] = 0;
    std::vector<int32_t> src((size_t)hs.nnz);
    hp.rowptr_i[0] = 0;
    std::vector<std::pair<int32_t, int32_t>> row;
    for (int64_t p = 0; p < nd; ++p) {
        const int32_t d = old_of_new[(size_t)p];
        row.clear();
        for (int32_t k = hs.rowptr_i[(size_t)d]; k < hs.rowptr_i[(size_t)d + 1]; ++k) row.push_back({new_of_old[(size_t)hs.colidx_i[(size_t)k]], k});
        std::sort(row.begin(), row.end());
        int32_t at = hp.rowptr_i[(size_t)p];
        for (const auto& e : row) hp.colidx_i[(size_t)at] = e.first, src[(size_t)at] = e.second, ++at;
        hp.rowptr_i[(size_t)p + 1] = at;
    }
    if (int rc = host_build_persist_layout(hp, true, G, lds_entries, pl, rows.data(), sym_mode, false)) return rc;
    for (int32_t& d : pl.slot_dof)
        if (d >= 0) d = old_of_new[(size_t)d];
    for (int32_t& k : pl.ell_src)
        if (k >= 0) k = src[(size_t)k];
    if (perm_out) *perm_out = std::move(perm);
    if (rows_out) *rows_out = std::move(rows);
    return FDAPDE_OK;
}

}
```

### fdapde-core_amd/csrc/internal.h

```cpp
#ifndef FDAPDE_INTERNAL_H
#define FDAPDE_INTERNAL_H

#include <cmath>
#include <cstdint>
#include <memory>
#include <new>
#include <string>
#include <utility>
#include <vector>

#include "../../include/fdapde_hip.h"

namespace fdapde_hip {

template <class T> struct NoInitAlloc : std::allocator<T> {
    template <class U> struct rebind { using other = NoInitAlloc<U>; };
    NoInitAlloc() = default;
    template <class U> NoInitAlloc(const NoInitAlloc<U>&) noexcept {}
    template <class U> void construct(U* p) noexcept { ::new (static_cast<void*>(p)) U; }
    template <class U, class... A> void construct(U* p, A&&... a) { ::new (static_cast<void*>(p)) U(std::forward<A>(a)...); }
};
template <class T> using hvec = std::vector<T, NoInitAlloc<T>>;

constexpr int kMaxBasis = 10;
constexpr int kMaxQuad = 6;
constexpr int kMaxTerms = 8;
constexpr int kSlice = 64;
constexpr int kAsmBlock = 256;

struct BasisTables {
    int M = 0, R = 0, nb = 0, nq = 0;
    double qn[kMaxQuad * 3] = {};
    double qw[kMaxQuad] = {};
    double psi[kMaxBasis * kMaxQuad] = {};
    double dpsi[kMaxBasis * kMaxQuad * 3] = {};
    double refnodes[kMaxBasis * 3] = {};
};
int build_basis_tables(int M, int R, BasisTables* t);
int n_basis_of(int M, int R);
int n_quadrature_of(int M, int R);

struct HostSpace {
    int M = 0, N = 0;
    int64_t n_nodes = 0, n_cells = 0;
    hvec<double> nodes;
    hvec<int32_t> cells;
    std::vector<uint8_t> node_bnd;
    int order = 0, nb = 0, nq = 0;
    int64_t n_dofs = 0, n_edges = 0;
    hvec<int32_t> dofs;
    std::vector<uint8_t> dof_bnd;
    hvec<double> dof_coords;
    hvec<int32_t> dof_e2i, dof_i2e, node_e2i, node_i2e, cell_e2i, cell_i2e;
    hvec<int32_t> rowptr_e, colidx_e;
    hvec<int32_t> rowptr_i, colidx_i, slot_i2e, diag_i;
    int64_t nnz = 0;
    int32_t max_row = 0;
    hvec<int32_t> cverts_i;
    hvec<int32_t> cdofs_i;
    hvec<double> vcoords_i;
    std::vector<uint8_t> dof_bnd_i;
    std::vector<int64_t> sl_off;
    int64_t n_slices = 0;
    int32_t max_slice_width = 0;
    hvec<int32_t> adj;
    hvec<int32_t> lane_row;
    int nbw = 0;
    hvec<uint32_t> slotw;
    std::vector<int32_t> blk_nnz_cap;
    int32_t max_blk_nnz = 0;
    std::vector<int64_t> bc_off;
    hvec<int32_t> bc_cell;
    hvec<uint16_t> bc_vert;
    std::vector<int64_t> bn_off;
    hvec<int32_t> bn_node;
    int32_t max_blk_nodes = 0, max_blk_cells = 0;
    int n_colours = 0;
    std::vector<int32_t> colour_off;
    std::vector<int32_t> colour_cells;
    std::vector<int32_t> rb_row;
    double setup_ms = 0;
};

constexpr int kSpmvNnz = 4096;

int host_set_mesh(HostSpace& hs, int M, int N, int64_t n_nodes, const double* nodes, int64_t n_cells,
                  const int32_t* cells, const uint8_t* bnd, std::string& err);
int host_build_space(HostSpace& hs, int order, std::string& err, int stop_after = 0);
int host_build_colouring(HostSpace& hs, std::string& err);
int host_build_solver_pattern_seg(const HostSpace& hs, bool use_bnd, int seg, int wrows, std::vector<int32_t>& rowptr_v,
                                  std::vector<int32_t>& colidx_s, std::vector<int32_t>& full2s, std::vector<int32_t>& vrow);
constexpr int kCodeRows = 32, kCodeWindow = 1 << 14;
int host_build_col16(int64_t n, const std::vector<int32_t>& rowptr, const std::vector<int32_t>& colidx, std::vector<uint16_t>& code,
                     std::vector<int32_t>& tbase, int64_t* n_wide);
int host_build_solver_pattern(const HostSpace& hs, bool use_bnd, std::vector<int32_t>& rowptr_s, std::vector<int32_t>& colidx_s,
                              std::vector<int32_t>& full2s);


struct CellPartitions {
    int32_t cells_per_part = 0, max_colours = 0;
    int64_t n_parts = 0;
    std::vector<int32_t> cell_list;
    std::vector<int32_t> colour_off;
    std::vector<uint8_t> dof_shared;
    std::vector<int32_t> slot_map;
};
int host_build_cell_partitions(const HostSpace& hs, int cells_per_part, CellPartitions& cp, std::string& err);
void host_build_slot_map(const HostSpace& hs, const int32_t* list, int64_t n, std::vector<int32_t>& out);

constexpr int kPersistT = 512;
constexpr int kPersistRmax = 16;
constexpr int kPersistRwide = 24;
inline int persist_rows_per_thread(int64_t rpw, int64_t max_halo, bool halo_free, bool sym) {
    constexpr int64_t T = kPersistT;
    int R = 2;
    while (R <= kPersistRmax && ((int64_t)R * T < rpw || (!halo_free && (int64_t)(R / 2) * T < max_halo))) R *= 2;
    if (R <= kPersistRmax) return R;
    if (!sym && (int64_t)kPersistRwide * T >= rpw && (halo_free || (int64_t)(kPersistRwide / 2) * T >= max_halo)) return kPersistRwide;
    return 0;
}
#ifdef __HIPCC__
__host__ __device__
#endif
inline bool persist_sym_owner(int32_t row, int32_t col) {
    const uint32_t lo = (uint32_t)(row < col ? row : col), hi = (uint32_t)(row < col ? col : row);
    const bool low_owns = ((((lo * 2654435761u) ^ (hi * 2246822519u)) >> 16) & 1u) != 0;
    return (low_owns ? lo : hi) == (uint32_t)row;
}
inline int64_t persist_want_workgroups(int64_t n_int, int64_t nnz_kept, int lds_entries, int32_t single_rows) {
    if (n_int <= single_rows) return 1;
    int64_t want = (n_int + 2047) / 2048;
    if (lds_entries > 0) {
        const int64_t fit = (nnz_kept + nnz_kept / 16 + lds_entries - 1) / lds_entries;
        if (fit > want) want = fit;
    }
    return want;
}
inline bool persist_want_sym(int sym_mode, int64_t nnz_kept, int G, int64_t rows_per_wg) {
    const bool plain_streams = 10.6 * (double)nnz_kept / (double)G + 16.0 * (double)rows_per_wg > 150e3;
    return sym_mode == 1 || (sym_mode == 2 && rows_per_wg > 2048 && plain_streams) || (sym_mode == 3 && plain_streams);
}
struct PersistLayout {
    int32_t single_rows = 2048;
    bool sym = false;
    bool bisect = false;
    int G = 0, R = 0, nsl = 0;
    int64_t n_int = 0;
    int64_t n_entries = 0;
    int64_t nnz = 0;
    int64_t nnz_full = 0;
    int64_t n_board = 0;
    int64_t n_imp = 0;
    int64_t n_drop = 0;
    int32_t max_imp = 0, max_exp = 0;
    int64_t max_block = 0;
    std::vector<int32_t> slot_dof;
    std::vector<int64_t> ell_off;
    std::vector<int32_t> sl_off;
    std::vector<uint16_t> ell_code;
    std::vector<int32_t> ell_src;
    std::vector<int32_t> exp_off;
    std::vector<uint16_t> exp_slot;
    std::vector<int32_t> imp_off;
    std::vector<int32_t> imp_pos;
    std::vector<int32_t> ghost_needed;
    std::vector<int32_t> wg_of, slot_of;
    std::vector<uint8_t> wg_late;
};
int host_build_persist_layout(const HostSpace& hs, bool use_bnd, int n_wg, int lds_entries, PersistLayout& pl, const int32_t* block_rows = nullptr,
                              int sym_mode = 0, bool balance = false, const int32_t* ghost_order = nullptr, bool allow_late = false);

inline double persist_bisect_span(int M, int N, int64_t n) {
    const double key_span = (double)((uint64_t(1) << (N == 3 ? 21 : 31)) - 1);
    double levels = std::floor(std::pow((double)(n > 1 ? n : 1), 1.0 / (double)(M >= 1 ? M : 1)) + 0.5) - 1.0;
    return levels < 1.0 ? 1.0 : (levels > key_span ? key_span : levels);
}
void host_bisect_quantise(int N, int64_t n, const double* pts_colmajor, const int32_t* i2e, double span, std::vector<uint32_t>& q);
int host_bisect_partition(int64_t n_int, const int32_t* cost, const uint32_t* qx, const uint32_t* qy, const uint32_t* qz, int G, std::vector<int32_t>& perm,
                          std::vector<int32_t>& block_rows);
int host_build_persist_layout_bisect(const HostSpace& hs, bool use_bnd, int G, int lds_entries, PersistLayout& pl, int sym_mode, const uint32_t* q,
                                     std::vector<int32_t>* perm_out = nullptr, std::vector<int32_t>* rows_out = nullptr);

}
#endif
```

### fdapde-core_amd/csrc/persist_engine.hip

```cpp
#include <algorithm>
#include <atomic>
#include <cstring>
#include <utility>

#include <unistd.h>

#include "engine.h"
#include "kernels_persist.h"
#include "kernels_persist_bicg.h"

static inline size_t dboard_offset(int64_t n_board) { return (2 * (size_t)n_board + 7) & ~(size_t)7; }

namespace fdapde_engine {

static int compare_dev_persist(fdapde_ctx* c, const PersistLayout& pl, const DevPersist& dp, const PersistLayout& ref);
int check_dev_persist(fdapde_ctx* c, int v, const PersistLayout& pl, const DevPersist& dp, const std::vector<int32_t>* block_rows, bool balance, int n_wg) {
    if (int rc = ensure_host(c, kHostPattern)) return rc;
    PersistLayout ref;
    ref.single_rows = pl.single_rows;
    if (host_build_persist_layout(c->hs, v == 1, n_wg, 12000, ref, block_rows ? block_rows->data() : nullptr,
                                  pl.sym ? 1 : 0, balance) != FDAPDE_OK) return fail(c, FDAPDE_EHIP, "set-up check: host persistent layout failed");
    return compare_dev_persist(c, pl, dp, ref);
}
int check_dev_persist_bisect(fdapde_ctx* c, int v, const PersistLayout& pl, const DevPersist& dp, const std::vector<int32_t>& perm, const std::vector<int32_t>& rows) {
    if (int rc = ensure_host(c, kHostPattern | kHostDofs)) return rc;
    std::vector<uint32_t> q;
    host_bisect_quantise(c->hs.N, c->hs.n_dofs, c->hs.dof_coords.data(), c->hs.dof_i2e.data(), persist_bisect_span(c->hs.M, c->hs.N, c->hs.n_dofs), q);
    PersistLayout ref;
    ref.single_rows = pl.single_rows;
    std::vector<int32_t> perm_h, rows_h;
    if (host_build_persist_layout_bisect(c->hs, v == 1, pl.G, 12000, ref, pl.sym ? 1 : 0, q.data(), &perm_h, &rows_h) != FDAPDE_OK)
        return fail(c, FDAPDE_EHIP, "set-up check: host bisection layout failed");
    const bool same_perm = perm == perm_h, same_rows = rows == rows_h;
    std::fprintf(stderr, "persist check %-9s: %s (%zu elements)\n", "bis_perm", same_perm ? "ok" : "MISMATCH", perm_h.size());
    std::fprintf(stderr, "persist check %-9s: %s (%zu elements)\n", "bis_rows", same_rows ? "ok" : "MISMATCH", rows_h.size());
    if (!same_perm || !same_rows) return fail(c, FDAPDE_EHIP, "FDAPDE_SETUP_CHECK: the device-built bisection differs from the host's (see stderr)");
    return compare_dev_persist(c, pl, dp, ref);
}
static int compare_dev_persist(fdapde_ctx* c, const PersistLayout& pl, const DevPersist& dp, const PersistLayout& ref) {
    int bad = 0;
    auto scalar = [&](const char* name, int64_t a, int64_t b) {
        if (a != b) std::fprintf(stderr, "persist check %-9s: MISMATCH %lld vs %lld\n", name, (long long)a, (long long)b), ++bad;
    };
    scalar("G", pl.G, ref.G), scalar("R", pl.R, ref.R), scalar("n_int", pl.n_int, ref.n_int), scalar("n_entries", pl.n_entries, ref.n_entries);
    scalar("nnz", pl.nnz, ref.nnz), scalar("n_board", pl.n_board, ref.n_board), scalar("max_imp", pl.max_imp, ref.max_imp), scalar("max_exp", pl.max_exp, ref.max_exp);
    auto cmp = [&](const char* name, const void* dev, const void* host, size_t bytes, size_t elem) {
        std::vector<unsigned char> tmp(bytes ? bytes : 1);
        if (bytes && hipMemcpy(tmp.data(), dev, bytes, hipMemcpyDeviceToHost) != hipSuccess) {
            ++bad;
            return;
        }
        size_t at = 0;
        while (at < bytes && tmp[at] == static_cast<const unsigned char*>(host)[at]) ++at;
        if (at < bytes) std::fprintf(stderr, "persist check %-9s: MISMATCH at element %zu of %zu\n", name, at / elem, bytes / elem), ++bad;
        else std::fprintf(stderr, "persist check %-9s: ok (%zu elements)\n", name, bytes / elem);
    };
    if (bad == 0) {
#define CMP(name, dptr, hvec_) cmp(name, dptr, (hvec_).data(), (hvec_).size() * sizeof((hvec_)[0]), sizeof((hvec_)[0]))
        CMP("slot_dof", dp.slot_dof, ref.slot_dof), CMP("ell_off", dp.ell_off, ref.ell_off), CMP("sl_off", dp.sl_off, ref.sl_off);
        CMP("ell_code", dp.ell_code, ref.ell_code), CMP("ell_src", dp.ell_src, ref.ell_src), CMP("exp_off", dp.exp_off, ref.exp_off);
        CMP("exp_slot", dp.exp_slot, ref.exp_slot), CMP("imp_off", dp.imp_off, ref.imp_off), CMP("imp_pos", dp.imp_pos, ref.imp_pos);
#undef CMP
    }
    if (bad) return fail(c, FDAPDE_EHIP, "FDAPDE_SETUP_CHECK: the device-built persistent layout differs from the host builder's (see stderr)");
    return FDAPDE_OK;
}

struct PersistNeeds {
    int S = 0, imp_cap = 0, exp_cap = 0;
    size_t fixed = 0;
    int64_t need = 0;
};
static PersistNeeds persist_needs(const PersistLayout& pl, bool host_built) {
    PersistNeeds n;
    n.S = pl.R * kPersistT;
    n.imp_cap = (pl.max_imp + 63) & ~63, n.exp_cap = (pl.max_exp + 63) & ~63;
    n.fixed = pl.sym ? 8 * (size_t)(n.S + n.imp_cap) + 8 * (size_t)n.S + 64 : 8 * (size_t)(n.S + n.imp_cap) + 4 * (size_t)n.imp_cap + 2 * (size_t)n.exp_cap + 64;
    if (pl.R > kPersistRmax) n.fixed = 8 * (size_t)(n.S + n.imp_cap) + 64;
    n.need = pl.max_block;
    for (int g = 0; g < pl.G && host_built; ++g) n.need = std::max<int64_t>(n.need, pl.ell_off[(size_t)g + 1] - pl.ell_off[(size_t)g]);
    n.need += 128;
    return n;
}

int build_persist_once(fdapde_ctx* c, int v, const std::vector<int32_t>* block_rows, bool balance) {
    fdapde_ctx::Persist& ps = c->ps[v];
    ps.ok = false;
    ps.ell_col.release();
    if (c->n_cu < 1) return FDAPDE_OK;
    const int32_t* brows = block_rows ? block_rows->data() : nullptr;
    const int n_wg = block_rows ? (int)block_rows->size() : (c->persist_max_wg > 0 ? std::min(c->persist_max_wg, c->n_cu) : c->n_cu);
    PersistLayout pl;
    DevPersist dp;
    DebugClock clk;
    const char* mode = std::getenv("FDAPDE_SETUP");
    bool on_device = !(mode && std::strcmp(mode, "host") == 0);
    if (c->hs.n_dofs <= c->persist_host_below && !(mode && std::strcmp(mode, "device") == 0)) on_device = false;
    double max_mb = 1024.0;
    if (const char* e = std::getenv("FDAPDE_PERSIST_MAX_MB")) max_mb = std::atof(e);
    const size_t lds_total = 160 * 1024 - 1024;
    size_t fixed = 0;
    int64_t need = 0;
    int imp_cap = 0, exp_cap = 0, S = 0;
    bool late_ok = c->persist_late != 0 && block_rows == nullptr;
    if (late_ok) on_device = false;
    int sym_mode = c->persist_sym == 2 ? 3 : c->persist_sym;
    if (c->persist_plain) sym_mode = 0;
    for (int attempt = 0; attempt < 2; ++attempt) {
        pl = PersistLayout{};
        pl.single_rows = c->persist_single_rows;
        int rc = FDAPDE_EUNSUPPORTED;
        if (on_device) {
            preload_wait(2);
            rc = dev_build_persist_layout(c->hs.n_dofs, c->hs.max_row, c->rowptr.p, c->colidx.p, c->bnd.p, v == 1, n_wg, 12000, 0, brows, sym_mode,
                                          balance, c->stream, pl, &dp, c->err);
            if (rc == FDAPDE_EUNSUPPORTED && c->hs.max_row > 255) on_device = false;
        }
        if (!on_device) {
            clk.mark("build_persist: (before ensure_host)");
            if (int rc2 = ensure_host(c, kHostPattern)) return rc2;
            clk.mark("build_persist: ensure_host");
            rc = host_build_persist_layout(c->hs, v == 1, n_wg, 12000, pl, brows, sym_mode, balance, nullptr, late_ok);
        }
        if (c->persist_plain && !late_ok && block_rows == nullptr && (rc == FDAPDE_EUNSUPPORTED || (rc == FDAPDE_OK && pl.R > 8)) &&
            (rc == FDAPDE_EUNSUPPORTED ? (c->hs.n_dofs + n_wg - 1) / n_wg <= 8 * kPersistT : (pl.n_int + pl.G - 1) / pl.G <= 8 * kPersistT) && attempt == 0) {
            dev_persist_release(&dp);
            late_ok = true, on_device = false;
            --attempt;
            continue;
        }
        if (rc == FDAPDE_EUNSUPPORTED && sym_mode != 0 && attempt == 0) {
            dev_persist_release(&dp);
            sym_mode = 0;
            continue;
        }
        if (rc == FDAPDE_EUNSUPPORTED) return FDAPDE_OK;
        if (rc) return rc;
        if (10.0 * (double)pl.n_entries > max_mb * 1e6) {
            dev_persist_release(&dp);
            return FDAPDE_OK;
        }
        {
            const PersistNeeds pn = persist_needs(pl, !on_device);
            S = pn.S, imp_cap = pn.imp_cap, exp_cap = pn.exp_cap, fixed = pn.fixed, need = pn.need;
        }
        if (pl.sym && fixed > lds_total && attempt == 0) {
            dev_persist_release(&dp);
            sym_mode = 0;
            continue;
        }
        if (c->persist_sym == 2 && pl.sym && attempt == 0 && pl.G == 1) {
            dev_persist_release(&dp);
            sym_mode = 0;
            continue;
        }
        if (c->persist_sym == 2 && pl.sym && attempt == 0) {
            const size_t fixed_plain = 8 * (size_t)(S + imp_cap) + 4 * (size_t)imp_cap + 2 * (size_t)exp_cap + 64;
            const size_t block_plain = (size_t)(1.03 * (double)pl.nnz_full / (double)pl.G) + 256;
            const bool plain_resident = pl.R < 16 && fixed_plain + 10 * block_plain <= lds_total;
            const bool sym_resident = fixed + 10 * (size_t)need <= lds_total;
            if (plain_resident || ((pl.n_int + pl.G - 1) / pl.G <= 2048 && !sym_resident)) {
                dev_persist_release(&dp);
                sym_mode = 0;
                continue;
            }
        }
        break;
    }
    clk.mark("build_persist: layout");
    ps.stream = fixed + 10 * (size_t)need > lds_total;
    if (fixed > lds_total || (pl.R >= 16 && !ps.stream) || (pl.R > kPersistRmax && (c->persist_plain || !c->persist_wide))) {
        dev_persist_release(&dp);
        return FDAPDE_OK;
    }
    const int part = c->persist_partition;
    const bool check = on_device && std::getenv("FDAPDE_SETUP_CHECK") != nullptr;
    if (check) {
        if (int rc2 = check_dev_persist(c, v, pl, dp, block_rows, balance, n_wg)) {
            dev_persist_release(&dp);
            return rc2;
        }
    }
    if (part != 0 && block_rows == nullptr && !late_ok && pl.G >= 2) {
        PersistLayout pl2;
        DevPersist dp2;
        pl2.single_rows = c->persist_single_rows;
        std::vector<int32_t> perm2, rows2;
        int rc2 = FDAPDE_EUNSUPPORTED;
        const size_t n_co = (size_t)c->hs.n_dofs * c->hs.N;
        if (on_device) {
            DBuf<double> coords_tmp;
            const double* coords = nullptr;
            if (c->hs.order == 1 && c->mesh_on_dev && c->mesh_nodes.n == n_co) coords = c->mesh_nodes.p;
            else if (c->coords_e.p && c->coords_e.n == n_co) coords = c->coords_e.p;
            else if (ensure_host(c, kHostDofs) == FDAPDE_OK && c->hs.dof_coords.size() == n_co &&
                     coords_tmp.upload(c->hs.dof_coords.data(), n_co, c->stream) == hipSuccess)
                coords = coords_tmp.p;
            if (coords)
                rc2 = dev_build_persist_layout_bisect(c->hs.n_dofs, c->hs.max_row, c->rowptr.p, c->colidx.p, c->bnd.p, v == 1, c->hs.M, c->hs.N, coords, c->dof_i2e.p, pl.G, 12000,
                                                      pl.sym ? 1 : 0, c->stream, pl2, &dp2, check ? &perm2 : nullptr, check ? &rows2 : nullptr, c->err);
            if (coords_tmp.p) (void)hipStreamSynchronize(c->stream);
        } else if (ensure_host(c, kHostPattern | kHostDofs) == FDAPDE_OK && c->hs.dof_coords.size() == n_co) {
            std::vector<uint32_t> q;
            host_bisect_quantise(c->hs.N, c->hs.n_dofs, c->hs.dof_coords.data(), c->hs.dof_i2e.data(), persist_bisect_span(c->hs.M, c->hs.N, c->hs.n_dofs), q);
            rc2 = host_build_persist_layout_bisect(c->hs, v == 1, pl.G, 12000, pl2, pl.sym ? 1 : 0, q.data());
        }
        if (rc2 != FDAPDE_OK) {
            (void)hipGetLastError();
            c->err.clear();
        }
        if (rc2 == FDAPDE_OK && check)
            if (int rc3 = check_dev_persist_bisect(c, v, pl2, dp2, perm2, rows2)) {
                dev_persist_release(&dp), dev_persist_release(&dp2);
                return rc3;
            }
        bool take = false;
        PersistNeeds pn2;
        bool stream2 = false;
        if (rc2 == FDAPDE_OK) {
            pn2 = persist_needs(pl2, !on_device);
            stream2 = pn2.fixed + 10 * (size_t)pn2.need > lds_total;
            auto bytes = [](const PersistLayout& l) {
                return 10.0 * (double)l.n_entries + 32.0 * (double)l.n_board + (l.R > kPersistRmax ? 16.0 * (double)l.n_int : 0.0);
            };
            const bool fits = 10.0 * (double)pl2.n_entries <= max_mb * 1e6 && pn2.fixed <= lds_total && !(pl2.R >= 16 && !stream2) &&
                              !(pl2.R > kPersistRmax && (c->persist_plain || !c->persist_wide));
            const bool same_form = pl2.sym == pl.sym && pl2.R <= pl.R && (!stream2 || ps.stream);
            take = fits && same_form && (part == 1 || bytes(pl2) < bytes(pl));
            if (std::getenv("FDAPDE_DEBUG_SETUP"))
                std::fprintf(stderr, "persistent CG layout %d: bisection %s: %.0f bytes per iteration against %.0f (entries %lld / %lld, board %lld / %lld, imports <= %d / %d, R %d / %d)\n",
                             v, take ? "taken" : "not taken", bytes(pl2), bytes(pl), (long long)pl2.n_entries, (long long)pl.n_entries, (long long)pl2.n_board,
                             (long long)pl.n_board, pl2.max_imp, pl.max_imp, pl2.R, pl.R);
        }
        if (take) {
            dev_persist_release(&dp);
            pl = std::move(pl2), dp = dp2;
            S = pn2.S, imp_cap = pn2.imp_cap, exp_cap = pn2.exp_cap, fixed = pn2.fixed, need = pn2.need, ps.stream = stream2;
            pl.bisect = true;
        } else
            dev_persist_release(&dp2);
        clk.mark("build_persist: bisection layout");
    }
    ps.lds_cap = ps.stream ? 0 : (int32_t)need, ps.imp_cap = imp_cap;
    ps.lds_bytes = fixed + (ps.stream ? 0 : 10 * (size_t)need);
    ps.exp_lds = pl.sym && ps.stream && pl.R <= kPersistRmax && ps.lds_bytes + 2 * (size_t)exp_cap + 1024 <= 160 * 1024 && c->persist_exp_lds;
    if (ps.exp_lds) ps.lds_bytes += 2 * (size_t)exp_cap;
    hipStream_t st = c->stream;
    if (on_device) {
        const size_t GS = (size_t)pl.G * S, n_alloc = (size_t)pl.n_entries + 256;
        adopt(ps.slot_dof, dp.slot_dof, GS), adopt(ps.ell_off, dp.ell_off, (size_t)pl.G + 1), adopt(ps.sl_off, dp.sl_off, (size_t)pl.G * (pl.nsl + 1));
        adopt(ps.ell_code, dp.ell_code, n_alloc), adopt(ps.ell_src, dp.ell_src, n_alloc), adopt(ps.exp_off, dp.exp_off, (size_t)pl.G + 1);
        adopt(ps.exp_slot, dp.exp_slot, (size_t)(pl.n_board ? pl.n_board : 1)), adopt(ps.imp_off, dp.imp_off, (size_t)pl.G + 1);
        adopt(ps.imp_pos, dp.imp_pos, (size_t)(pl.n_imp ? pl.n_imp : 1));
    } else {
        HIPCHK(c, ps.slot_dof.upload(pl.slot_dof.data(), pl.slot_dof.size(), st));
        HIPCHK(c, ps.ell_off.upload(pl.ell_off.data(), pl.ell_off.size(), st));
        HIPCHK(c, ps.sl_off.upload(pl.sl_off.data(), pl.sl_off.size(), st));
        HIPCHK(c, ps.ell_code.alloc(pl.ell_code.size() + 256));
        HIPCHK(c, hipMemsetAsync(ps.ell_code.p, 0, sizeof(uint16_t) * (pl.ell_code.size() + 256), st));
        HIPCHK(c, hipMemcpyAsync(ps.ell_code.p, pl.ell_code.data(), sizeof(uint16_t) * pl.ell_code.size(), hipMemcpyHostToDevice, st));
        HIPCHK(c, ps.ell_src.upload(pl.ell_src.data(), pl.ell_src.size(), st));
        HIPCHK(c, ps.exp_off.upload(pl.exp_off.data(), pl.exp_off.size(), st));
        HIPCHK(c, ps.exp_slot.upload(pl.exp_slot.data(), pl.exp_slot.size(), st));
        HIPCHK(c, ps.imp_off.upload(pl.imp_off.data(), pl.imp_off.size(), st));
        HIPCHK(c, ps.imp_pos.upload(pl.imp_pos.data(), pl.imp_pos.size(), st));
    }
    if (late_ok && !pl.wg_late.empty()) HIPCHK(c, ps.wg_late.upload(pl.wg_late.data(), pl.wg_late.size(), st));
    else ps.wg_late.release();
    HIPCHK(c, ps.ell_val.alloc((size_t)pl.n_entries + 256));
    HIPCHK(c, hipMemsetAsync(ps.ell_val.p, 0, sizeof(double) * ((size_t)pl.n_entries + 256), st));
    HIPCHK(c, ps.board.alloc(dboard_offset(pl.n_board) + 2 * (size_t)pl.G * 8 + 8));
    HIPCHK(c, hipMemsetAsync(ps.board.p, 0, sizeof(unsigned long long) * ps.board.n, st));
    ps.epoch_next = 0, ps.attr_set = nullptr;
    ps.board_cols.release();
    HIPCHK(c, ps.amax.alloc(1));
    HIPCHK(c, c->persist_stats.alloc(4 * 1024));
    HIPCHK(c, hipStreamSynchronize(st));
    clk.mark("build_persist: uploads + allocs");
    if (std::getenv("FDAPDE_DEBUG_SETUP"))
        std::fprintf(stderr, "persistent CG layout %d (%s-built): %d workgroups x %d rows/thread, %lld interior rows, %lld entries (%lld stored, %.1f %% padding), "
                     "LDS %zu B (%s%s, largest block %lld), imports <= %d, exports <= %d, board %lld\n", v, on_device ? "device" : "host", pl.G, pl.R,
                     (long long)pl.n_int, (long long)pl.n_entries, (long long)pl.nnz,
                     100.0 * (double)(pl.n_entries - pl.nnz) / (double)(pl.n_entries > 0 ? pl.n_entries : 1), ps.lds_bytes,
                     ps.stream ? "blocks stream" : "blocks resident", pl.sym ? (pl.bisect ? ", symmetric storage, bisection blocks" : ", symmetric storage") : (pl.bisect ? ", bisection blocks" : ""), (long long)need, pl.max_imp, pl.max_exp, (long long)pl.n_board);
    pl.slot_dof = {}, pl.ell_code = {}, pl.ell_src = {}, pl.exp_slot = {}, pl.imp_pos = {}, pl.sl_off = {}, pl.ell_off = {};
    ps.meta = std::move(pl);
    ps.filled = false, ps.ok = true;
    return FDAPDE_OK;
}

int launch_persist(fdapde_ctx* c, fdapde_ctx::Persist& ps, PersistArgs& a, bool dist = false, bool bicg = false) {
    hipStream_t st = c->stream;
    a.G = ps.meta.G, a.nsl = ps.meta.nsl, a.imp_cap = ps.imp_cap, a.lds_cap = ps.lds_cap;
    a.gather_waves = c->persist_gather_waves, a.poll_sleep = c->persist_poll_sleep;
    a.slot_dof = ps.slot_dof.p, a.ell_off = ps.ell_off.p, a.sl_off = ps.sl_off.p, a.ell_code = ps.ell_code.p;
    a.ell_val = ps.ell_val.p, a.exp_off = ps.exp_off.p, a.exp_slot = ps.exp_slot.p, a.imp_off = ps.imp_off.p, a.imp_pos = ps.imp_pos.p;
    if (!dist && a.n_cols <= 1) a.pboard = ps.board.p, a.dboard = ps.board.p + dboard_offset(ps.meta.n_board);
    if (!dist) a.wg_late = ps.wg_late.p;
    a.exp_lds = (!dist && !bicg && ps.exp_lds) ? 1 : 0;
    a.amax_bits = ps.amax.p, a.max_len = c->hs.max_row, a.stats = c->persist_stats.p;
    a.timeout_ticks = c->persist_timeout_us * 100, a.debug_stall_it = c->persist_debug_stall, a.pf_steps = c->persist_prefetch;
    if (!dist && ps.epoch_next > 0xC0000000u - 2u * (uint32_t)a.maxit) {
        HIPCHK(c, hipMemsetAsync(ps.board.p, 0, sizeof(unsigned long long) * ps.board.n, st));
        if (ps.board_cols.p) HIPCHK(c, hipMemsetAsync(ps.board_cols.p, 0, sizeof(unsigned long long) * ps.board_cols.n, st));
        ps.epoch_next = 0;
    }
    a.epoch0 = ps.epoch_next;
    if (a.time_phases) HIPCHK(c, hipMemsetAsync(c->persist_stats.p, 0, 4 * (size_t)a.G * sizeof(double), st));
    HIPCHK(c, hipEventRecord(c->ev_p0, st));
    void* kargs[] = {&a};
#define PERSIST_GO(R_, ST_, SY_) PERSIST_GO_D(R_, ST_, SY_, false)
#define PERSIST_GO_D(R_, ST_, SY_, DI_)                                                                                         \
    do {                                                                                                                        \
        const void* fn = reinterpret_cast<const void*>(&k_cg_persist<R_, ST_, SY_, DI_>);                                       \
        if (ps.attr_set != fn) {                                                                                                \
            DebugClock clk2;                                                                                                    \
            HIPCHK(c, hipFuncSetAttribute(fn, hipFuncAttributeMaxDynamicSharedMemorySize, (int)ps.lds_bytes));                  \
            clk2.mark("launch_persist: hipFuncSetAttribute");                                                                   \
            int per_cu = 0;                                                                                                     \
            HIPCHK(c, hipOccupancyMaxActiveBlocksPerMultiprocessor(&per_cu, fn, kPersistT, ps.lds_bytes));                      \
            clk2.mark("launch_persist: occupancy query");                                                                       \
            if ((int64_t)per_cu * c->n_cu < (int64_t)a.G) return FDAPDE_EUNSUPPORTED;    \
            ps.attr_set = fn, ps.per_cu = per_cu;                                                                               \
        }                                                                                                                       \
        const unsigned ncol = a.n_cols > 1 ? (unsigned)a.n_cols : 1u;                                                           \
        if ((int64_t)ps.per_cu * c->n_cu < (int64_t)a.G * ncol) return FDAPDE_EUNSUPPORTED;                                     \
        if (c->persist_coop) HIPCHK(c, hipLaunchCooperativeKernel(fn, dim3(a.G, ncol), dim3(kPersistT), kargs, (unsigned)ps.lds_bytes, st)); \
        else hipLaunchKernelGGL((k_cg_persist<R_, ST_, SY_, DI_>), dim3(a.G, ncol), dim3(kPersistT), ps.lds_bytes, st, a);      \
    } while (0)
#define PERSIST_GO2(R_, ST_)                                                                                                    \
    do {                                                                                                                        \
        if (ps.meta.sym) PERSIST_GO(R_, ST_, true);                                                                             \
        else PERSIST_GO(R_, ST_, false);                                                                                        \
    } while (0)
#define PERSIST_GOD(R_, ST_)                                                                                                    \
    do {                                                                                                                        \
        if (ps.meta.sym) PERSIST_GO_D(R_, ST_, true, true);                                                                     \
        else PERSIST_GO_D(R_, ST_, false, true);                                                                                \
    } while (0)
#define BICG_GO(R_, ST_, DI_)                                                                                                   \
    do {                                                                                                                        \
        const void* fn = reinterpret_cast<const void*>(&k_bicg_persist<R_, ST_, DI_>);                                          \
        if (ps.attr_set != fn) {                                                                                                \
            HIPCHK(c, hipFuncSetAttribute(fn, hipFuncAttributeMaxDynamicSharedMemorySize, (int)ps.lds_bytes));                  \
            int per_cu = 0;                                                                                                     \
            HIPCHK(c, hipOccupancyMaxActiveBlocksPerMultiprocessor(&per_cu, fn, kPersistT, ps.lds_bytes));                      \
            if ((int64_t)per_cu * c->n_cu < (int64_t)a.G) return FDAPDE_EUNSUPPORTED;                                           \
            ps.attr_set = fn, ps.per_cu = per_cu;                                                                               \
        }                                                                                                                       \
        const unsigned ncol = a.n_cols > 1 ? (unsigned)a.n_cols : 1u;                                                           \
        if ((int64_t)ps.per_cu * c->n_cu < (int64_t)a.G * ncol) return FDAPDE_EUNSUPPORTED;                                     \
        hipLaunchKernelGGL((k_bicg_persist<R_, ST_, DI_>), dim3(a.G, ncol), dim3(kPersistT), ps.lds_bytes, st, a);              \
    } while (0)
#define BICG_GO2(R_, ST_)                                                                                                       \
    do {                                                                                                                        \
        if (dist) BICG_GO(R_, ST_, true);                                                                                       \
        else BICG_GO(R_, ST_, false);                                                                                           \
    } while (0)
    if (bicg) {
        if (ps.meta.sym) return FDAPDE_EUNSUPPORTED;
        if (ps.stream) switch (ps.meta.R) {
            case 2: BICG_GO2(2, true); break;
            case 4: BICG_GO2(4, true); break;
            case 8: BICG_GO2(8, true); break;
            default: return FDAPDE_EUNSUPPORTED;
            }
        else switch (ps.meta.R) {
            case 2: BICG_GO2(2, false); break;
            case 4: BICG_GO2(4, false); break;
            case 8: BICG_GO2(8, false); break;
            default: return FDAPDE_EUNSUPPORTED;
            }
    } else if (dist) {
        if (ps.stream) switch (ps.meta.R) {
            case 2: PERSIST_GOD(2, true); break;
            case 4: PERSIST_GOD(4, true); break;
            case 8: PERSIST_GOD(8, true); break;
            case 16: PERSIST_GOD(16, true); break;
            default: return FDAPDE_EUNSUPPORTED;
            }
        else switch (ps.meta.R) {
            case 2: PERSIST_GOD(2, false); break;
            case 4: PERSIST_GOD(4, false); break;
            case 8: PERSIST_GOD(8, false); break;
            default: return FDAPDE_EUNSUPPORTED;
            }
    } else if (ps.stream) switch (ps.meta.R) {
        case 2: PERSIST_GO2(2, true); break;
        case 4: PERSIST_GO2(4, true); break;
        case 8: PERSIST_GO2(8, true); break;
        case 16: PERSIST_GO2(16, true); break;
        case kPersistRwide:
            if (ps.meta.sym || a.n_cols > 1 || a.direct) return FDAPDE_EUNSUPPORTED;
            if (c->persist_xs.n < (size_t)ps.meta.G * kPersistRwide * kPersistT) HIPCHK(c, c->persist_xs.alloc((size_t)ps.meta.G * kPersistRwide * kPersistT));
            a.x_slots = c->persist_xs.p;
            {
                const void* fn = c->persist_wide_gj == 12 ? reinterpret_cast<const void*>(&k_cg_persist<kPersistRwide, true, false, false, 12>)
                               : c->persist_wide_gj == 4  ? reinterpret_cast<const void*>(&k_cg_persist<kPersistRwide, true, false, false, 4>)
                                                          : reinterpret_cast<const void*>(&k_cg_persist<kPersistRwide, true, false, false, 6>);
                if (ps.attr_set != fn) {
                    HIPCHK(c, hipFuncSetAttribute(fn, hipFuncAttributeMaxDynamicSharedMemorySize, (int)ps.lds_bytes));
                    int per_cu = 0;
                    HIPCHK(c, hipOccupancyMaxActiveBlocksPerMultiprocessor(&per_cu, fn, kPersistT, ps.lds_bytes));
                    if ((int64_t)per_cu * c->n_cu < (int64_t)a.G) return FDAPDE_EUNSUPPORTED;
                    ps.attr_set = fn, ps.per_cu = per_cu;
                }
                if (c->persist_wide_gj == 12) hipLaunchKernelGGL((k_cg_persist<kPersistRwide, true, false, false, 12>), dim3(a.G), dim3(kPersistT), ps.lds_bytes, st, a);
                else if (c->persist_wide_gj == 4) hipLaunchKernelGGL((k_cg_persist<kPersistRwide, true, false, false, 4>), dim3(a.G), dim3(kPersistT), ps.lds_bytes, st, a);
                else hipLaunchKernelGGL((k_cg_persist<kPersistRwide, true, false, false, 6>), dim3(a.G), dim3(kPersistT), ps.lds_bytes, st, a);
            }
            break;
        default: return FDAPDE_EUNSUPPORTED;
        }
    else switch (ps.meta.R) {
        case 2: PERSIST_GO2(2, false); break;
        case 4: PERSIST_GO2(4, false); break;
        default: PERSIST_GO2(8, false); break;
        }
#undef BICG_GO2
#undef BICG_GO
#undef PERSIST_GOD
#undef PERSIST_GO2
#undef PERSIST_GO_D
#undef PERSIST_GO
    HIPCHK(c, hipGetLastError());
    HIPCHK(c, hipEventRecord(c->ev_p1, st));
    return FDAPDE_OK;
}

int build_persist(fdapde_ctx* c, int v) {
    fdapde_ctx::Persist& ps = c->ps[v];
    if (ps.tried && ps.built_plain != (c->persist_plain != 0) && (ps.built_plain || (ps.ok && ps.meta.sym) || !ps.ok)) ps.tried = false;
    if (ps.tried) return FDAPDE_OK;
    ps.built_plain = c->persist_plain != 0;
    ps.tried = true;
    if (int rc = build_persist_once(c, v, nullptr, c->persist_balance != 0)) return rc;
    if (!ps.ok && c->persist_balance) return build_persist_once(c, v, nullptr, false);
// ... 649 lines not shown
```

### include/fdapde_hip.h

```cpp
#ifndef FDAPDE_HIP_H
#define FDAPDE_HIP_H

#include <stdint.h>

#ifdef __cplusplus
extern "C" {
#endif

#define FDAPDE_ABI_VERSION 5

enum {
    FDAPDE_OK = 0,
    FDAPDE_EINVAL = 1,
    FDAPDE_ENOMEM = 2,
    FDAPDE_ENODEVICE = 3,
    FDAPDE_EHIP = 4,
    FDAPDE_ENOTINIT = 5,
    FDAPDE_ENOCONV = 6,
    FDAPDE_EUNSUPPORTED = 7,
    FDAPDE_ERCCL = 8
};

enum { FDAPDE_LAPLACIAN = 0, FDAPDE_DIFFUSION = 1, FDAPDE_ADVECTION = 2, FDAPDE_REACTION = 3, FDAPDE_DT = 4 };

typedef struct {
    int32_t kind;
    int32_t space_varying;
    double coef;
    double cst[9];
    const double *data;
} fdapde_term;

enum { FDAPDE_SOLVER_AUTO = 0, FDAPDE_SOLVER_CG = 1, FDAPDE_SOLVER_BICGSTAB = 2, FDAPDE_SOLVER_CG_SR = 3, FDAPDE_SOLVER_CG_FUSED = 4,
       FDAPDE_SOLVER_GMRES = 5 ,
       FDAPDE_SOLVER_DENSE = 6 ,
       FDAPDE_SOLVER_PMG = 7 ,
       FDAPDE_SOLVER_AMG = 8  };
enum { FDAPDE_ASSEMBLY_ROWS = 0, FDAPDE_ASSEMBLY_ATOMIC = 1, FDAPDE_ASSEMBLY_COLOURED = 2, FDAPDE_ASSEMBLY_PARTITIONED = 3,
       FDAPDE_ASSEMBLY_WAVE = 4 };
enum { FDAPDE_MAT_STIFF = 0, FDAPDE_MAT_MASS = 1 };

typedef struct {
    int32_t method;
    int32_t maxit;
    double rtol;
    int32_t assembly;
    int32_t check_every;
    int32_t time_spmv;
} fdapde_options;

typedef struct {
    int32_t iters;
    int32_t converged;
    double relres;
    double t_assemble_ms;
    double t_solve_ms;
    double t_setup_ms;
    double spmv_avg_ms;
    int32_t spmv_timed;
    int32_t method_used;
    int32_t persistent;
    double gather_avg_ms;
    double update_avg_ms;
    double spmv_mean_ms;
    double launch_ms;
} fdapde_info;

typedef struct fdapde_ctx fdapde_ctx;

int fdapde_abi_version(void);
int fdapde_device_count(void);
int fdapde_ctx_create(int device, fdapde_ctx **ctx);
void fdapde_ctx_destroy(fdapde_ctx *ctx);
int fdapde_ctx_clone(const fdapde_ctx *src, fdapde_ctx **out);
int fdapde_ctx_create_multi(const int32_t *devices, int32_t n_devices, fdapde_ctx **ctx);
int fdapde_ctx_devices(const fdapde_ctx *ctx, int32_t *n_devices, int32_t *devices, int32_t *form, double *t_partition_ms,
                       double *t_rank_setup_ms);
const char *fdapde_last_error(const fdapde_ctx *ctx);
const char *fdapde_status_string(int status);

int fdapde_mesh_upload(fdapde_ctx *ctx, int M, int N, int64_t n_nodes, const double *nodes_colmajor, int64_t n_cells,
                       const int32_t *cells_rowmajor, const uint8_t *boundary_nodes);

int fdapde_topology_build(fdapde_ctx *ctx, int64_t *n_facets, int64_t *n_edges);
int fdapde_topology_get(fdapde_ctx *ctx, int32_t *neighbors, int32_t *cell_facets, int32_t *facet_nodes, int32_t *facet_cells,
                        uint8_t *facet_boundary, int32_t *edge_nodes, uint8_t *edge_boundary, int32_t *face_edges);

int fdapde_dofs_build(fdapde_ctx *ctx, int order, int64_t *n_dofs);
int fdapde_dofs_get(const fdapde_ctx *ctx, int32_t *dofs_rowmajor, uint8_t *boundary_dofs, double *dof_coords_colmajor);
int fdapde_dofs_set_boundary(fdapde_ctx *ctx, const uint8_t *boundary_dofs);
int fdapde_sizes(const fdapde_ctx *ctx, int64_t *n_dofs, int64_t *nnz, int32_t *n_basis, int32_t *n_quadrature,
                 int64_t *n_edges);
int fdapde_pattern_get(const fdapde_ctx *ctx, int32_t *rowptr, int32_t *colidx);
int fdapde_quadrature_nodes(fdapde_ctx *ctx, double *out_colmajor);

int fdapde_set_operator(fdapde_ctx *ctx, int32_t n_terms, const fdapde_term *terms);
int fdapde_set_forcing(fdapde_ctx *ctx, const double *f_q, int32_t n_cols);
int fdapde_set_dirichlet(fdapde_ctx *ctx, const double *g);

int fdapde_init(fdapde_ctx *ctx, const fdapde_options *opt);
int fdapde_assemble_operator(fdapde_ctx *ctx, int32_t which, int32_t n_terms, const fdapde_term *terms, int32_t assembly);

int fdapde_solver_prepare(fdapde_ctx *ctx, int32_t with_dirichlet);
int fdapde_solve(fdapde_ctx *ctx, const fdapde_options *opt, fdapde_info *info);

int fdapde_solve_parabolic(fdapde_ctx *ctx, const fdapde_options *opt, int32_t n_times, double delta_t,
                           const double *initial_condition, const double *dirichlet, double *solution, fdapde_info *info);

int fdapde_lin_compute(fdapde_ctx *ctx, int32_t which, const double *values, int32_t symmetric);
int fdapde_lin_solve(fdapde_ctx *ctx, const fdapde_options *opt, const double *b, int32_t n_rhs, double *x, fdapde_info *info);

int fdapde_eval_pointwise(fdapde_ctx *ctx, int64_t n_locs, const double *locs_colmajor, int32_t *cell_ids, double *values);
int fdapde_cell_integrals(fdapde_ctx *ctx, double *measure, double *psi_int);

int fdapde_matrix_values(fdapde_ctx *ctx, int32_t which, double *values);
int fdapde_lump(fdapde_ctx *ctx, int32_t which, double *diag);
int fdapde_force(fdapde_ctx *ctx, double *force);
int fdapde_solution(fdapde_ctx *ctx, double *solution);
int fdapde_info_get(const fdapde_ctx *ctx, fdapde_info *info);

int fdapde_spmv(fdapde_ctx *ctx, int32_t which, const double *x, double *y);
int fdapde_bench_spmv(fdapde_ctx *ctx, int32_t reps, double *avg_ms, double *algorithmic_bytes);
int fdapde_solver_layout(fdapde_ctx *ctx, int32_t with_dirichlet, int64_t *n_interior, int64_t *nnz_interior,
                         double *streamed_bytes);
int fdapde_solver_layout_kind(fdapde_ctx *ctx, int32_t with_dirichlet, int32_t *kind, int32_t *symmetric_storage,
                              int32_t *workgroups, int32_t *rows_per_thread);
int fdapde_solver_layout_partition(fdapde_ctx *ctx, int32_t with_dirichlet, int32_t *partition);
typedef int (*fdapde_allreduce_fn)(void *user, double *host_buf, int64_t count);
int fdapde_comm_init_callback(fdapde_ctx *ctx, int32_t world, int32_t rank, fdapde_allreduce_fn fn, void *user);
int fdapde_comm_unique_id(void *out128);
int fdapde_comm_init(fdapde_ctx *ctx, int32_t world, int32_t rank, const void *unique_id128);
int fdapde_comm_allreduce(fdapde_ctx *ctx, double *host_inout, int32_t n, int32_t op);
int fdapde_comm_count(fdapde_ctx *ctx, int32_t *ranks);
const char *fdapde_comm_library(void);
int fdapde_halo_setup(fdapde_ctx *ctx, int64_t n_if_global, int64_t n_if_local, const int32_t *local_dof,
                      const int32_t *if_index, const uint8_t *owned);
typedef int (*fdapde_exchange_fn)(void *user, int32_t n_peers, const int32_t *peer_rank, const int64_t *peer_off, const double *send,
                                  double *recv);
int fdapde_comm_set_exchange_callback(fdapde_ctx *ctx, fdapde_exchange_fn fn, void *user);
int fdapde_halo_setup_peers(fdapde_ctx *ctx, int32_t n_peers, const int32_t *peer_rank, const int64_t *peer_off,
                            const int32_t *peer_dof, const uint8_t *owned);

int fdapde_rowdist_setup(fdapde_ctx *ctx, const int64_t *dof_key, const int32_t *dof_owner);

int fdapde_partition_build(fdapde_ctx *ctx, int32_t world, int32_t form);
int fdapde_partition_sizes(const fdapde_ctx *ctx, int32_t rank, int64_t *n_nodes, int64_t *n_cells);
int fdapde_partition_get(fdapde_ctx *ctx, int32_t rank, double *nodes_colmajor, int32_t *cells_rowmajor, uint8_t *boundary_nodes,
                         int64_t *node_ids, int64_t *cell_ids, int32_t *node_owner);
int fdapde_partition_whole(fdapde_ctx *ctx, int32_t *cell_rank, int32_t *node_owner, uint64_t *node_ranks);
int fdapde_partition_peers(fdapde_ctx *ctx, int32_t rank, int32_t *n_peers, int32_t *peer_rank, int64_t *peer_off, int32_t *peer_node,
                           uint8_t *owned, int64_t *n_shared);

int fdapde_tune(fdapde_ctx *ctx, const char *key, int32_t value);
void *fdapde_stream(fdapde_ctx *ctx);
int fdapde_synchronize(fdapde_ctx *ctx);

#ifdef __cplusplus
}
#endif
#endif
```

Measured before the change: 117.7 million.

## Rebalance bisection partition blocks by measured per-block bytes in persistent CG

Adds iterative load-balancing rounds to the recursive-bisection partition of the persistent CG layout. After an initial bisection, it prices each workgroup block's bytes per iteration, rescales row costs by each block's share, and re-bisects, keeping a round only if the largest block shrinks. The aim is to cut the straggler block that bounds each persistent-kernel iteration. The cost is extra setup work (repeated sorts and layout builds), plus new tuning, query and debug plumbing.

New measurement: 118.9 million (median of 6 runs). No clear change (+1.0%).

```diff
diff --git a/fdapde-core_amd/capi.py b/fdapde-core_amd/capi.py
--- a/fdapde-core_amd/capi.py
+++ b/fdapde-core_amd/capi.py
@@ -40,7 +40,7 @@
     "fdapde_info_get", "fdapde_spmv", "fdapde_bench_spmv", "fdapde_tune", "fdapde_stream", "fdapde_synchronize",
     "fdapde_comm_unique_id", "fdapde_comm_init", "fdapde_halo_setup", "fdapde_solve_parabolic",
     "fdapde_lin_compute", "fdapde_lin_solve", "fdapde_eval_pointwise", "fdapde_cell_integrals", "fdapde_comm_init_callback", "fdapde_comm_set_exchange_callback", "fdapde_halo_setup_peers",
-    "fdapde_solver_layout", "fdapde_topology_build", "fdapde_topology_get", "fdapde_comm_allreduce", "fdapde_comm_library", "fdapde_solver_layout_kind", "fdapde_solver_layout_partition", "fdapde_rowdist_setup", "fdapde_ctx_clone", "fdapde_comm_count",
+    "fdapde_solver_layout", "fdapde_topology_build", "fdapde_topology_get", "fdapde_comm_allreduce", "fdapde_comm_library", "fdapde_solver_layout_kind", "fdapde_solver_layout_partition", "fdapde_solver_layout_balance", "fdapde_rowdist_setup", "fdapde_ctx_clone", "fdapde_comm_count",
     "fdapde_ctx_create_multi", "fdapde_ctx_devices", "fdapde_partition_build", "fdapde_partition_sizes", "fdapde_partition_get", "fdapde_partition_whole",
     "fdapde_partition_peers",
 ]
@@ -456,6 +456,11 @@
         self._check(self.lib.fdapde_solver_layout_partition(self._ctx, 1 if with_dirichlet else 0, C.byref(p)))
         return p.value
 
+    def solver_layout_balance(self, with_dirichlet=True):
+        r, mx, mean = C.c_int32(), C.c_int64(), C.c_int64()
+        self._check(self.lib.fdapde_solver_layout_balance(self._ctx, 1 if with_dirichlet else 0, C.byref(r), C.byref(mx), C.byref(mean)))
+        return dict(rounds_kept=r.value, max_block_bytes=mx.value, mean_block_bytes=mean.value)
+
     @staticmethod
     def comm_unique_id() -> bytes:
         buf = C.create_string_buffer(128)
diff --git a/fdapde-core_amd/csrc/capi.hip b/fdapde-core_amd/csrc/capi.hip
--- a/fdapde-core_amd/csrc/capi.hip
+++ b/fdapde-core_amd/csrc/capi.hip
@@ -266,6 +266,16 @@
     if (partition) *partition = (kind == 2 || kind == 3) && ps.ok ? (ps.meta.bisect ? 1 : 0) : -1;
     return FDAPDE_OK;
 }
+int fdapde_solver_layout_balance(fdapde_ctx* c, int32_t with_dirichlet, int32_t* rounds_kept, int64_t* max_block_bytes, int64_t* mean_block_bytes) {
+    int32_t kind = 0;
+    if (int rc = fdapde_solver_layout_kind(c, with_dirichlet, &kind, nullptr, nullptr, nullptr)) return rc;
+    const fdapde_ctx::Persist& ps = c->ps[with_dirichlet ? 1 : 0];
+    const bool have = (kind == 2 || kind == 3) && ps.ok && ps.meta.G > 0;
+    if (rounds_kept) *rounds_kept = have ? ps.meta.bal_kept : -1;
+    if (max_block_bytes) *max_block_bytes = have ? ps.meta.bal_max : 0;
+    if (mean_block_bytes) *mean_block_bytes = have ? ps.meta.bal_sum / ps.meta.G : 0;
+    return FDAPDE_OK;
+}
 int fdapde_solve(fdapde_ctx* c, const fdapde_options* opt, fdapde_info* info) {
     if (!c) return FDAPDE_EINVAL;
     if (c->group && opt && opt->method == FDAPDE_SOLVER_AMG) return fdapde_engine::fail(c, FDAPDE_EUNSUPPORTED, "FDAPDE_SOLVER_AMG takes one-GPU contexts, not a multi-device context");
@@ -485,6 +495,10 @@
         c->persist_partition = value;
         for (auto& ps : c->ps) ps.tried = ps.ok = ps.filled = false;
     }
+    else if (k == "persist_balance_rounds" && value >= 0 && value <= fdapde_hip::kPersistBalanceMaxRounds) {
+        c->persist_balance_rounds = value;
+        for (auto& ps : c->ps) ps.tried = ps.ok = ps.filled = false;
+    }
     else if (k == "persist_late" && (value == 0 || value == 1)) {
         c->persist_late = value;
         for (auto& ps : c->ps) ps.tried = ps.ok = ps.filled = false;
diff --git a/fdapde-core_amd/csrc/context.h b/fdapde-core_amd/csrc/context.h
--- a/fdapde-core_amd/csrc/context.h
+++ b/fdapde-core_amd/csrc/context.h
@@ -383,6 +383,7 @@
     bool defer_end_sync = false;
     int persist_single_rows = 2048;
     int persist_prefetch = 1;
+    int persist_balance_rounds = 2;
     int persist_partition = 2;
     int persist_late = 0;
     int persist_plain = 0;
diff --git a/fdapde-core_amd/csrc/dev_persist.h b/fdapde-core_amd/csrc/dev_persist.h
--- a/fdapde-core_amd/csrc/dev_persist.h
+++ b/fdapde-core_amd/csrc/dev_persist.h
@@ -22,7 +22,8 @@
 
 int dev_build_persist_layout_bisect(int64_t nd, int32_t max_row, const int32_t* d_rowptr, const int32_t* d_colidx, const uint8_t* d_bnd, bool use_bnd, int M,
                                     int N, const double* d_coords, const int32_t* d_i2e, int G, int lds_entries, int sym_mode, void* stream, PersistLayout& pl,
-                                    DevPersist* out, std::vector<int32_t>* perm_out, std::vector<int32_t>* rows_out, std::string& err);
+                                    DevPersist* out, std::vector<int32_t>* perm_out, std::vector<int32_t>* rows_out, std::string& err,
+                                    PersistBalance* bal = nullptr);
 
 void dev_persist_preload();
 }
diff --git a/fdapde-core_amd/csrc/dev_persist.hip b/fdapde-core_amd/csrc/dev_persist.hip
--- a/fdapde-core_amd/csrc/dev_persist.hip
+++ b/fdapde-core_amd/csrc/dev_persist.hip
@@ -814,6 +814,20 @@
     const int64_t i = (int64_t)blockIdx.x * blockDim.x + threadIdx.x;
     if (i < n && v[i] >= 0) v[i] = map[v[i]];
 }
+__global__ void k_bis_iota(int64_t n, int32_t* ord) {
+    const int64_t i = (int64_t)blockIdx.x * blockDim.x + threadIdx.x;
+    if (i < n) ord[i] = (int32_t)i;
+}
+__global__ void k_bis_cost_unit(int64_t n, const int32_t* cost, int32_t* cs) {
+    const int64_t i = (int64_t)blockIdx.x * blockDim.x + threadIdx.x;
+    if (i < n) cs[i] = kPersistCostUnit * cost[i];
+}
+__global__ void k_bis_scale_cost(int64_t n_int, const int32_t* ord, const int32_t* segb, int G, const int64_t* wb, int64_t sum_b, int32_t* cs) {
+    const int64_t p = (int64_t)blockIdx.x * blockDim.x + threadIdx.x;
+    if (p >= n_int) return;
+    const int32_t row = ord[p];
+    cs[row] = persist_balance_cost(cs[row], wb[wg_of_irow(segb, G, p)], G, sum_b);
+}
 inline int bits_for(int64_t n) {
     int b = 1;
     while ((int64_t(1) << b) < n) ++b;
@@ -824,7 +838,7 @@
 
 int dev_build_persist_layout_bisect(int64_t nd, int32_t max_row, const int32_t* d_rowptr, const int32_t* d_colidx, const uint8_t* d_bnd, bool use_bnd, int M,
                                     int N, const double* d_coords, const int32_t* d_i2e, int G, int lds_entries, int sym_mode, void* stream, PersistLayout& pl,
-                                    DevPersist* out, std::vector<int32_t>* perm_out, std::vector<int32_t>* rows_out, std::string& err) {
+                                    DevPersist* out, std::vector<int32_t>* perm_out, std::vector<int32_t>* rows_out, std::string& err, PersistBalance* bal) {
     hipStream_t st = static_cast<hipStream_t>(stream);
     if (G < 2 || G > kPersistT || nd < 1 || max_row > 255 || N < 1 || N > 3) return FDAPDE_EUNSUPPORTED;
     Arena arena;
@@ -874,45 +888,47 @@
     DP_CHK(ext.alloc(6 * (size_t)G));
     const double span = persist_bisect_span(M, N, nd);
     hipLaunchKernelGGL(k_bis_rows, dim3(grid_of(nd)), dim3(256), 0, st, nd, n_int, N, keep.p, irow_scan.p, len.p, d_i2e, d_coords, bb.p, span, cost.p, q.p, ord_a.p);
-    std::vector<int32_t> segg{G};
-    {
-        const int32_t b0[2] = {0, (int32_t)n_int};
-        DP_CHK(hipMemcpyAsync(seg_a.p, b0, sizeof(b0), hipMemcpyHostToDevice, st));
-        DP_CHK(hipMemcpyAsync(sgg_a.p, segg.data(), sizeof(int32_t), hipMemcpyHostToDevice, st));
+    int32_t *ord = ord_a.p, *segb = seg_a.p;
+    auto bisect = [&](const int32_t* costp, std::vector<int32_t>& h_rows) -> int {
+        int32_t *ord_n = ord_b.p, *segb_n = seg_b.p, *sgg = sgg_a.p, *sgg_n = sgg_b.p;
+        ord = ord_a.p, segb = seg_a.p;
+        hipLaunchKernelGGL(k_bis_iota, dim3(grid_of(n_int)), dim3(256), 0, st, n_int, ord);
+        std::vector<int32_t> segg{G};
+        {
+            const int32_t b0[2] = {0, (int32_t)n_int};
+            DP_CHK(hipMemcpyAsync(segb, b0, sizeof(b0), hipMemcpyHostToDevice, st));
+            DP_CHK(hipMemcpyAsync(sgg, segg.data(), sizeof(int32_t), hipMemcpyHostToDevice, st));
+            DP_CHK(hipStreamSynchronize(st));
+        }
+        while (*std::max_element(segg.begin(), segg.end()) > 1) {
+            const int nseg = (int)segg.size();
+            DP_CHK(hipMemsetAsync(ext.p, 0xff, sizeof(uint32_t) * 3 * (size_t)nseg, st));
+            DP_CHK(hipMemsetAsync(ext.p + 3 * (size_t)G, 0, sizeof(uint32_t) * 3 * (size_t)nseg, st));
+            hipLaunchKernelGGL(k_bis_extent, dim3((unsigned)((n_int + 256 * kBisPer - 1) / (256 * kBisPer))), dim3(256), 0, st, n_int, ord, segb, nseg, q.p, ext.p, ext.p + 3 * (size_t)G);
+            hipLaunchKernelGGL(k_bis_keys, dim3(grid_of(n_int)), dim3(256), 0, st, n_int, ord, segb, sgg, nseg, q.p, ext.p, ext.p + 3 * (size_t)G, key_a.p);
+            if (int rc = sort_pairs(sc, key_a.p, key_b.p, ord, ord_n, n_int, 31 + bits_for(nseg), st, err)) return rc;
+            hipLaunchKernelGGL(k_bis_gather_cost, dim3(grid_of(n_int + 1)), dim3(256), 0, st, n_int, ord_n, costp, c2.p);
+            if (int rc = exclusive_sum(sc, c2.p, pre.p, n_int + 1, st, err)) return rc;
+            hipLaunchKernelGGL(k_bis_split, dim3(1), dim3(512), 0, st, nseg, segb, sgg, pre.p, segb_n, sgg_n);
+            std::swap(ord, ord_n), std::swap(segb, segb_n), std::swap(sgg, sgg_n);
+            std::vector<int32_t> ng;
+            for (int32_t g : segg) {
+                if (g > 1) ng.push_back(g / 2), ng.push_back(g - g / 2);
+                else ng.push_back(1);
+            }
+            segg.swap(ng);
+        }
+        DP_CHK(hipGetLastError());
+        std::vector<int32_t> h_b((size_t)G + 1);
+        h_rows.resize((size_t)G);
+        DP_CHK(hipMemcpyAsync(h_b.data(), segb, sizeof(int32_t) * ((size_t)G + 1), hipMemcpyDeviceToHost, st));
         DP_CHK(hipStreamSynchronize(st));
-    }
-    int32_t *ord = ord_a.p, *ord_n = ord_b.p, *segb = seg_a.p, *segb_n = seg_b.p, *sgg = sgg_a.p, *sgg_n = sgg_b.p;
-    while (*std::max_element(segg.begin(), segg.end()) > 1) {
-        const int nseg = (int)segg.size();
-        DP_CHK(hipMemsetAsync(ext.p, 0xff, sizeof(uint32_t) * 3 * (size_t)nseg, st));
-        DP_CHK(hipMemsetAsync(ext.p + 3 * (size_t)G, 0, sizeof(uint32_t) * 3 * (size_t)nseg, st));
-        hipLaunchKernelGGL(k_bis_extent, dim3((unsigned)((n_int + 256 * kBisPer - 1) / (256 * kBisPer))), dim3(256), 0, st, n_int, ord, segb, nseg, q.p, ext.p, ext.p + 3 * (size_t)G);
-        hipLaunchKernelGGL(k_bis_keys, dim3(grid_of(n_int)), dim3(256), 0, st, n_int, ord, segb, sgg, nseg, q.p, ext.p, ext.p + 3 * (size_t)G, key_a.p);
-        if (int rc = sort_pairs(sc, key_a.p, key_b.p, ord, ord_n, n_int, 31 + bits_for(nseg), st, err)) return rc;
-        hipLaunchKernelGGL(k_bis_gather_cost, dim3(grid_of(n_int + 1)), dim3(256), 0, st, n_int, ord_n, cost.p, c2.p);
-        if (int rc = exclusive_sum(sc, c2.p, pre.p, n_int + 1, st, err)) return rc;
-        hipLaunchKernelGGL(k_bis_split, dim3(1), dim3(512), 0, st, nseg, segb, sgg, pre.p, segb_n, sgg_n);
-        std::swap(ord, ord_n), std::swap(segb, segb_n), std::swap(sgg, sgg_n);
-        std::vector<int32_t> ng;
-        for (int32_t g : segg) {
-            if (g > 1) ng.push_back(g / 2), ng.push_back(g - g / 2);
-            else ng.push_back(1);
-        }
-        segg.swap(ng);
-    }
-    DP_CHK(hipGetLastError());
-    std::vector<int32_t> h_b((size_t)G + 1), h_rows((size_t)G);
-    DP_CHK(hipMemcpyAsync(h_b.data(), segb, sizeof(int32_t) * ((size_t)G + 1), hipMemcpyDeviceToHost, st));
-    DP_CHK(hipStreamSynchronize(st));
-    for (int g = 0; g < G; ++g) {
-        h_rows[(size_t)g] = h_b[(size_t)g + 1] - h_b[(size_t)g];
-        if (h_rows[(size_t)g] < 1) return FDAPDE_EUNSUPPORTED;
-    }
-    if (perm_out) {
-        perm_out->resize((size_t)n_int);
-        DP_CHK(hipMemcpyAsync(perm_out->data(), ord, sizeof(int32_t) * (size_t)n_int, hipMemcpyDeviceToHost, st));
-        DP_CHK(hipStreamSynchronize(st));
-    }
+        for (int g = 0; g < G; ++g) {
+            h_rows[(size_t)g] = h_b[(size_t)g + 1] - h_b[(size_t)g];
+            if (h_rows[(size_t)g] < 1) return FDAPDE_EUNSUPPORTED;
+        }
+        return FDAPDE_OK;
+    };
     Tmp<int32_t> pos_of_row, new_of_old, old_of_new, len_new, rowptr_new, colidx_new, src_a, src_new;
     Tmp<uint8_t> bnd_new;
     Tmp<uint64_t> ek_a, ek_b;
@@ -927,31 +943,122 @@
     DP_CHK(ek_a.alloc((size_t)nnz));
     DP_CHK(ek_b.alloc((size_t)nnz));
     DP_CHK(bnd_new.alloc((size_t)nd));
-    hipLaunchKernelGGL(k_bis_invert, dim3(grid_of(n_int)), dim3(256), 0, st, n_int, ord, pos_of_row.p);
-    DP_CHK(hipMemsetAsync(len_new.p + nd, 0, sizeof(int32_t), st));
-    hipLaunchKernelGGL(k_bis_numbering, dim3(grid_of(nd)), dim3(256), 0, st, nd, n_int, keep.p, irow_scan.p, pos_of_row.p, d_rowptr, new_of_old.p, old_of_new.p,
-                       len_new.p);
-    if (int rc = exclusive_sum(sc, len_new.p, rowptr_new.p, nd + 1, st, err)) return rc;
-    hipLaunchKernelGGL(k_bis_entries, dim3(grid_of(nd)), dim3(256), 0, st, nd, d_rowptr, d_colidx, new_of_old.p, rowptr_new.p, ek_a.p, src_a.p);
-    if (nnz > 0) {
-        if (int rc = sort_pairs(sc, ek_a.p, ek_b.p, src_a.p, src_new.p, nnz, 32 + bits_for(nd), st, err)) return rc;
-        hipLaunchKernelGGL(k_low32, dim3(grid_of(nnz)), dim3(256), 0, st, nnz, ek_b.p, colidx_new.p);
-    }
-    DP_CHK(hipMemsetAsync(colidx_new.p + nnz, 0, 2 * sizeof(int32_t), st));
-    DP_CHK(hipMemsetAsync(bnd_new.p, 0, (size_t)n_int, st));
-    if (nd > n_int) DP_CHK(hipMemsetAsync(bnd_new.p + n_int, 1, (size_t)(nd - n_int), st));
-    DP_CHK(hipGetLastError());
+    auto layout = [&](const std::vector<int32_t>& h_rows, PersistLayout& plx, DevPersist& ox) -> int {
+        hipLaunchKernelGGL(k_bis_invert, dim3(grid_of(n_int)), dim3(256), 0, st, n_int, ord, pos_of_row.p);
+        DP_CHK(hipMemsetAsync(len_new.p + nd, 0, sizeof(int32_t), st));
+        hipLaunchKernelGGL(k_bis_numbering, dim3(grid_of(nd)), dim3(256), 0, st, nd, n_int, keep.p, irow_scan.p, pos_of_row.p, d_rowptr, new_of_old.p, old_of_new.p,
+                           len_new.p);
+        if (int rc = exclusive_sum(sc, len_new.p, rowptr_new.p, nd + 1, st, err)) return rc;
+        hipLaunchKernelGGL(k_bis_entries, dim3(grid_of(nd)), dim3(256), 0, st, nd, d_rowptr, d_colidx, new_of_old.p, rowptr_new.p, ek_a.p, src_a.p);
+        if (nnz > 0) {
+            if (int rc = sort_pairs(sc, ek_a.p, ek_b.p, src_a.p, src_new.p, nnz, 32 + bits_for(nd), st, err)) return rc;
+            hipLaunchKernelGGL(k_low32, dim3(grid_of(nnz)), dim3(256), 0, st, nnz, ek_b.p, colidx_new.p);
+        }
+        DP_CHK(hipMemsetAsync(colidx_new.p + nnz, 0, 2 * sizeof(int32_t), st));
+        DP_CHK(hipMemsetAsync(bnd_new.p, 0, (size_t)n_int, st));
+        if (nd > n_int) DP_CHK(hipMemsetAsync(bnd_new.p + n_int, 1, (size_t)(nd - n_int), st));
+        DP_CHK(hipGetLastError());
+        DevPersist o;
+        if (int rc = dev_build_persist_layout(nd, max_row, rowptr_new.p, colidx_new.p, bnd_new.p, true, G, lds_entries, 0, h_rows.data(), sym_mode, false, stream, plx, &o,
+                                              err))
+            return rc;
+        const int64_t n_slots = (int64_t)plx.G * plx.R * kPersistT, n_ent = plx.n_entries + 256;
+        hipLaunchKernelGGL(k_bis_map_back, dim3(grid_of(n_slots)), dim3(256), 0, st, n_slots, old_of_new.p, o.slot_dof);
+        hipLaunchKernelGGL(k_bis_map_back, dim3(grid_of(n_ent)), dim3(256), 0, st, n_ent, src_new.p, o.ell_src);
+        if (hipGetLastError() != hipSuccess || hipStreamSynchronize(st) != hipSuccess) {
+            dev_persist_release(&o);
+            err = "bisection layout: mapping back failed";
+            return FDAPDE_EHIP;
+        }
+        ox = o;
+        return FDAPDE_OK;
+    };
+    auto fetch_perm = [&](std::vector<int32_t>& v) -> int {
+        v.resize((size_t)n_int);
+        DP_CHK(hipMemcpyAsync(v.data(), ord, sizeof(int32_t) * (size_t)n_int, hipMemcpyDeviceToHost, st));
+        DP_CHK(hipStreamSynchronize(st));
+        return FDAPDE_OK;
+    };
+    std::vector<int32_t> h_rows;
+    if (int rc = bisect(cost.p, h_rows)) return rc;
+    if (perm_out)
+        if (int rc = fetch_perm(*perm_out)) return rc;
     DevPersist o;
-    if (int rc = dev_build_persist_layout(nd, max_row, rowptr_new.p, colidx_new.p, bnd_new.p, true, G, lds_entries, 0, h_rows.data(), sym_mode, false, stream, pl, &o,
-                                          err))
-        return rc;
-    const int64_t n_slots = (int64_t)pl.G * pl.R * kPersistT, n_ent = pl.n_entries + 256;
-    hipLaunchKernelGGL(k_bis_map_back, dim3(grid_of(n_slots)), dim3(256), 0, st, n_slots, old_of_new.p, o.slot_dof);
-    hipLaunchKernelGGL(k_bis_map_back, dim3(grid_of(n_ent)), dim3(256), 0, st, n_ent, src_new.p, o.ell_src);
-    if (hipGetLastError() != hipSuccess || hipStreamSynchronize(st) != hipSuccess) {
-        dev_persist_release(&o);
-        err = "bisection layout: mapping back failed";
-        return FDAPDE_EHIP;
+    if (int rc = layout(h_rows, pl, o)) return rc;
+    if (bal) {
+        std::vector<int64_t> B, h_ell((size_t)G + 1);
+        std::vector<int32_t> h_exp((size_t)G + 1), h_imp((size_t)G + 1);
+        auto price = [&](const PersistLayout& l, const DevPersist& d, int64_t& mx, int64_t& sum, PersistForm& f, bool& fits) -> int {
+            DP_CHK(hipMemcpyAsync(h_ell.data(), d.ell_off, sizeof(int64_t) * ((size_t)G + 1), hipMemcpyDeviceToHost, st));
+            DP_CHK(hipMemcpyAsync(h_exp.data(), d.exp_off, sizeof(int32_t) * ((size_t)G + 1), hipMemcpyDeviceToHost, st));
+            DP_CHK(hipMemcpyAsync(h_imp.data(), d.imp_off, sizeof(int32_t) * ((size_t)G + 1), hipMemcpyDeviceToHost, st));
+            DP_CHK(hipStreamSynchronize(st));
+            persist_block_bytes(G, h_ell.data(), h_exp.data(), h_imp.data(), B, mx, sum);
+            bool stream_ = false;
+            fits = persist_layout_fits(l, persist_needs(l, false), bal->fit, stream_);
+            f.sym = l.sym, f.R = l.R, f.stream = stream_;
+            return FDAPDE_OK;
+        };
+        PersistForm held;
+        bool fits0 = false;
+        bal->tried = bal->kept = 0;
+        if (int rc = price(pl, o, bal->max_bytes0, bal->sum_bytes0, held, fits0)) {
+            dev_persist_release(&o);
+            return rc;
+        }
+        bal->max_bytes = bal->max_bytes0, bal->sum_bytes = bal->sum_bytes0;
+        if (pl.G == G && persist_balance_wanted(*bal, pl, held, fits0)) {
+            const int64_t bytes0 = persist_layout_bytes(pl);
+            int64_t cur_sum = bal->sum_bytes0;
+            auto rounds = [&]() -> int {
+                Tmp<int32_t> cs;
+                Tmp<int64_t> wb;
+                DP_CHK(cs.alloc((size_t)n_int));
+                DP_CHK(wb.alloc((size_t)G));
+                hipLaunchKernelGGL(k_bis_cost_unit, dim3(grid_of(n_int)), dim3(256), 0, st, n_int, cost.p, cs.p);
+                for (int r = 1; r <= std::min(bal->rounds, kPersistBalanceMaxRounds); ++r) {
+                    DP_CHK(hipMemcpyAsync(wb.p, B.data(), sizeof(int64_t) * (size_t)G, hipMemcpyHostToDevice, st));
+                    hipLaunchKernelGGL(k_bis_scale_cost, dim3(grid_of(n_int)), dim3(256), 0, st, n_int, ord, segb, G, wb.p, cur_sum, cs.p);
+                    DP_CHK(hipStreamSynchronize(st));
+                    std::vector<int32_t> rows_c;
+                    if (int rc = bisect(cs.p, rows_c)) return rc;
+                    PersistLayout cand;
+                    cand.single_rows = pl.single_rows;
+                    DevPersist oc;
+                    if (int rc = layout(rows_c, cand, oc)) return rc;
+                    if (cand.G != G) {
+                        dev_persist_release(&oc);
+                        return FDAPDE_EUNSUPPORTED;
+                    }
+                    bal->tried = r;
+                    int64_t mx = 0, sum = 0;
+                    PersistForm fc;
+                    bool fits = false;
+                    if (int rc = price(cand, oc, mx, sum, fc, fits)) {
+                        dev_persist_release(&oc);
+                        return rc;
+                    }
+                    cur_sum = sum;
+                    bool keep_it = sum >= 1 && persist_balance_keeps(*bal, cand, fc, fits, mx, held, bal->max_bytes, bytes0);
+                    std::vector<int32_t> perm_c;
+                    if (keep_it && perm_out && fetch_perm(perm_c) != FDAPDE_OK) keep_it = false;
+                    if (keep_it) {
+                        dev_persist_release(&o);
+                        o = oc, pl = std::move(cand), h_rows = rows_c, held = fc;
+                        if (perm_out) perm_out->swap(perm_c);
+                        bal->kept = r, bal->max_bytes = mx, bal->sum_bytes = sum;
+                    } else
+                        dev_persist_release(&oc);
+                    if (sum < 1) break;
+                }
+                return FDAPDE_OK;
+            };
+            if (rounds() != FDAPDE_OK) {
+                (void)hipGetLastError();
+                err.clear();
+            }
+        }
+        pl.bal_kept = bal->kept, pl.bal_max = bal->max_bytes, pl.bal_sum = bal->sum_bytes;
     }
     if (rows_out) *rows_out = std::move(h_rows);
     *out = o;
diff --git a/fdapde-core_amd/csrc/host_bisect.cpp b/fdapde-core_amd/csrc/host_bisect.cpp
--- a/fdapde-core_amd/csrc/host_bisect.cpp
+++ b/fdapde-core_amd/csrc/host_bisect.cpp
@@ -65,7 +65,7 @@
 }
 
 int host_build_persist_layout_bisect(const HostSpace& hs, bool use_bnd, int G, int lds_entries, PersistLayout& pl, int sym_mode, const uint32_t* q,
-                                     std::vector<int32_t>* perm_out, std::vector<int32_t>* rows_out) {
+                                     std::vector<int32_t>* perm_out, std::vector<int32_t>* rows_out, PersistBalance* bal) {
     const int64_t nd = hs.n_dofs;
     auto dropped = [&](int64_t d) { return use_bnd && hs.dof_bnd_i[(size_t)d] != 0; };
     std::vector<int32_t> irow_dof, cost;
@@ -81,40 +81,87 @@
         for (int a = 0; a < 3; ++a) qi[a].push_back(q[(size_t)a * (size_t)nd + (size_t)d]);
     }
     const int64_t n_int = (int64_t)irow_dof.size();
+    auto build = [&](const std::vector<int32_t>& cst, PersistLayout& out, std::vector<int32_t>& perm, std::vector<int32_t>& rows) -> int {
+        if (int rc = host_bisect_partition(n_int, cst.data(), qi[0].data(), qi[1].data(), qi[2].data(), G, perm, rows)) return rc;
+        std::vector<int32_t> old_of_new((size_t)nd), new_of_old((size_t)nd);
+        for (int64_t p = 0; p < n_int; ++p) old_of_new[(size_t)p] = irow_dof[(size_t)perm[(size_t)p]];
+        {
+            int64_t p = n_int;
+            for (int64_t d = 0; d < nd; ++d)
+                if (dropped(d)) old_of_new[(size_t)p++] = (int32_t)d;
+        }
+        for (int64_t p = 0; p < nd; ++p) new_of_old[(size_t)old_of_new[(size_t)p]] = (int32_t)p;
+        HostSpace hp;
+        hp.n_dofs = nd, hp.nnz = hs.nnz, hp.max_row = hs.max_row;
+        hp.dof_bnd_i.assign((size_t)nd, 0);
+        for (int64_t p = n_int; p < nd; ++p) hp.dof_bnd_i[(size_t)p] = 1;
+        hp.rowptr_i.resize((size_t)nd + 1);
+        hp.colidx_i.resize((size_t)hs.nnz + 2);
+        hp.colidx_i[(size_t)hs.nnz] = hp.colidx_i[(size_t)hs.nnz + 1] = 0;
+        std::vector<int32_t> src((size_t)hs.nnz);
+        hp.rowptr_i[0] = 0;
+        std::vector<std::pair<int32_t, int32_t>> row;
+        for (int64_t p = 0; p < nd; ++p) {
+            const int32_t d = old_of_new[(size_t)p];
+            row.clear();
+            for (int32_t k = hs.rowptr_i[(size_t)d]; k < hs.rowptr_i[(size_t)d + 1]; ++k) row.push_back({new_of_old[(size_t)hs.colidx_i[(size_t)k]], k});
+            std::sort(row.begin(), row.end());
+            int32_t at = hp.rowptr_i[(size_t)p];
+            for (const auto& e : row) hp.colidx_i[(size_t)at] = e.first, src[(size_t)at] = e.second, ++at;
+            hp.rowptr_i[(size_t)p + 1] = at;
+        }
+        if (int rc = host_build_persist_layout(hp, true, G, lds_entries, out, rows.data(), sym_mode, false)) return rc;
+        for (int32_t& d : out.slot_dof)
+            if (d >= 0) d = old_of_new[(size_t)d];
+        for (int32_t& k : out.ell_src)
+            if (k >= 0) k = src[(size_t)k];
+        return FDAPDE_OK;
+    };
     std::vector<int32_t> perm, rows;
-    if (int rc = host_bisect_partition(n_int, cost.data(), qi[0].data(), qi[1].data(), qi[2].data(), G, perm, rows)) return rc;
-    std::vector<int32_t> old_of_new((size_t)nd), new_of_old((size_t)nd);
-    for (int64_t p = 0; p < n_int; ++p) old_of_new[(size_t)p] = irow_dof[(size_t)perm[(size_t)p]];
-    {
-        int64_t p = n_int;
-        for (int64_t d = 0; d < nd; ++d)
-            if (dropped(d)) old_of_new[(size_t)p++] = (int32_t)d;
+    if (int rc = build(cost, pl, perm, rows)) return rc;
+    if (bal) {
+        std::vector<int64_t> B;
+        auto price = [&](const PersistLayout& l, int64_t& mx, int64_t& sum, PersistForm& f) {
+            persist_block_bytes(l.G, l.ell_off.data(), l.exp_off.data(), l.imp_off.data(), B, mx, sum);
+            bool stream = false;
+            const bool fits = persist_layout_fits(l, persist_needs(l, true), bal->fit, stream);
+            f.sym = l.sym, f.R = l.R, f.stream = stream;
+            return fits;
+        };
+        PersistForm held;
+        bal->tried = bal->kept = 0;
+        const bool fits0 = price(pl, bal->max_bytes0, bal->sum_bytes0, held);
+        bal->max_bytes = bal->max_bytes0, bal->sum_bytes = bal->sum_bytes0;
+        if (persist_balance_wanted(*bal, pl, held, fits0)) {
+            const int64_t bytes0 = persist_layout_bytes(pl);
+            std::vector<int32_t> cs((size_t)n_int), cperm = perm, crows = rows, nperm, nrows;
+            for (int64_t i = 0; i < n_int; ++i) cs[(size_t)i] = kPersistCostUnit * cost[(size_t)i];
+            int64_t cur_sum = bal->sum_bytes0;
+            for (int r = 1; r <= std::min(bal->rounds, kPersistBalanceMaxRounds); ++r) {
+                int64_t p = 0;
+                for (int g = 0; g < G; ++g)
+                    for (int32_t k = 0; k < crows[(size_t)g]; ++k, ++p) {
+                        int32_t& c = cs[(size_t)cperm[(size_t)p]];
+                        c = persist_balance_cost(c, B[(size_t)g], G, cur_sum);
+                    }
+                PersistLayout cand;
+                cand.single_rows = pl.single_rows;
+                if (build(cs, cand, nperm, nrows) != FDAPDE_OK || cand.G != G) break;
+                bal->tried = r;
+                int64_t mx = 0, sum = 0;
+                PersistForm fc;
+                const bool fits = price(cand, mx, sum, fc);
+                cur_sum = sum;
+                if (sum < 1) break;
+                if (persist_balance_keeps(*bal, cand, fc, fits, mx, held, bal->max_bytes, bytes0)) {
+                    pl = std::move(cand), perm = nperm, rows = nrows, held = fc;
+                    bal->kept = r, bal->max_bytes = mx, bal->sum_bytes = sum;
+                }
+                cperm.swap(nperm), crows.swap(nrows);
+            }
+        }
+        pl.bal_kept = bal->kept, pl.bal_max = bal->max_bytes, pl.bal_sum = bal->sum_bytes;
     }
-    for (int64_t p = 0; p < nd; ++p) new_of_old[(size_t)old_of_new[(size_t)p]] = (int32_t)p;
-    HostSpace hp;
-    hp.n_dofs = nd, hp.nnz = hs.nnz, hp.max_row = hs.max_row;
-    hp.dof_bnd_i.assign((size_t)nd, 0);
-    for (int64_t p = n_int; p < nd; ++p) hp.dof_bnd_i[(size_t)p] = 1;
-    hp.rowptr_i.resize((size_t)nd + 1);
-    hp.colidx_i.resize((size_t)hs.nnz + 2);
-    hp.colidx_i[(size_t)hs.nnz] = hp.colidx_i[(size_t)hs.nnz + 1] = 0;
-    std::vector<int32_t> src((size_t)hs.nnz);
-    hp.rowptr_i[0] = 0;
-    std::vector<std::pair<int32_t, int32_t>> row;
-    for (int64_t p = 0; p < nd; ++p) {
-        const int32_t d = old_of_new[(size_t)p];
-        row.clear();
-        for (int32_t k = hs.rowptr_i[(size_t)d]; k < hs.rowptr_i[(size_t)d + 1]; ++k) row.push_back({new_of_old[(size_t)hs.colidx_i[(size_t)k]], k});
-        std::sort(row.begin(), row.end());
-        int32_t at = hp.rowptr_i[(size_t)p];
-        for (const auto& e : row) hp.colidx_i[(size_t)at] = e.first, src[(size_t)at] = e.second, ++at;
-        hp.rowptr_i[(size_t)p + 1] = at;
-    }
-    if (int rc = host_build_persist_layout(hp, true, G, lds_entries, pl, rows.data(), sym_mode, false)) return rc;
-    for (int32_t& d : pl.slot_dof)
-        if (d >= 0) d = old_of_new[(size_t)d];
-    for (int32_t& k : pl.ell_src)
-        if (k >= 0) k = src[(size_t)k];
     if (perm_out) *perm_out = std::move(perm);
     if (rows_out) *rows_out = std::move(rows);
     return FDAPDE_OK;
diff --git a/fdapde-core_amd/csrc/internal.h b/fdapde-core_amd/csrc/internal.h
--- a/fdapde-core_amd/csrc/internal.h
+++ b/fdapde-core_amd/csrc/internal.h
@@ -1,6 +1,7 @@
 #ifndef FDAPDE_INTERNAL_H
 #define FDAPDE_INTERNAL_H
 
+#include <algorithm>
 #include <cmath>
 #include <cstdint>
 #include <memory>
@@ -154,6 +155,8 @@
     int64_t n_drop = 0;
     int32_t max_imp = 0, max_exp = 0;
     int64_t max_block = 0;
+    int bal_kept = 0;
+    int64_t bal_max = 0, bal_sum = 0;
     std::vector<int32_t> slot_dof;
     std::vector<int64_t> ell_off;
     std::vector<int32_t> sl_off;
@@ -178,8 +181,83 @@
 void host_bisect_quantise(int N, int64_t n, const double* pts_colmajor, const int32_t* i2e, double span, std::vector<uint32_t>& q);
 int host_bisect_partition(int64_t n_int, const int32_t* cost, const uint32_t* qx, const uint32_t* qy, const uint32_t* qz, int G, std::vector<int32_t>& perm,
                           std::vector<int32_t>& block_rows);
+constexpr int64_t kPersistBytesEntry = 10, kPersistBytesExport = 16, kPersistBytesImport = 16;
+constexpr int32_t kPersistCostUnit = 64, kPersistCostMax = 1 << 20;
+constexpr int kPersistBalanceMaxRounds = 8;
+#ifdef __HIPCC__
+__host__ __device__
+#endif
+inline int32_t persist_balance_cost(int32_t cost, int64_t block_bytes, int64_t G, int64_t sum_bytes) {
+    const int64_t v = (int64_t)cost * block_bytes * G / sum_bytes;
+    return (int32_t)(v < 1 ? 1 : (v > kPersistCostMax ? kPersistCostMax : v));
+}
+inline void persist_block_bytes(int G, const int64_t* ell_off, const int32_t* exp_off, const int32_t* imp_off, std::vector<int64_t>& B, int64_t& max_b, int64_t& sum_b) {
+    B.resize((size_t)G), max_b = sum_b = 0;
+    for (int g = 0; g < G; ++g) {
+        B[(size_t)g] = kPersistBytesEntry * (ell_off[g + 1] - ell_off[g]) + kPersistBytesExport * (int64_t)(exp_off[g + 1] - exp_off[g]) +
+                       kPersistBytesImport * (int64_t)(imp_off[g + 1] - imp_off[g]);
+        max_b = std::max(max_b, B[(size_t)g]), sum_b += B[(size_t)g];
+    }
+}
+struct PersistNeeds {
+    int S = 0, imp_cap = 0, exp_cap = 0;
+    size_t fixed = 0;
+    int64_t need = 0;
+};
+inline PersistNeeds persist_needs(const PersistLayout& pl, bool host_built) {
+    PersistNeeds n;
+    n.S = pl.R * kPersistT;
+    n.imp_cap = (pl.max_imp + 63) & ~63, n.exp_cap = (pl.max_exp + 63) & ~63;
+    n.fixed = pl.sym ? 8 * (size_t)(n.S + n.imp_cap) + 8 * (size_t)n.S + 64 : 8 * (size_t)(n.S + n.imp_cap) + 4 * (size_t)n.imp_cap + 2 * (size_t)n.exp_cap + 64;
+    if (pl.R > kPersistRmax) n.fixed = 8 * (size_t)(n.S + n.imp_cap) + 64;
+    n.need = pl.max_block;
+    for (int g = 0; g < pl.G && host_built; ++g) n.need = std::max<int64_t>(n.need, pl.ell_off[(size_t)g + 1] - pl.ell_off[(size_t)g]);
+    n.need += 128;
+    return n;
+}
+struct PersistFit {
+    size_t lds_total = 160 * 1024 - 1024;
+    double max_mb = 1024.0;
+    bool plain = false, wide = true;
+};
+inline int64_t persist_layout_bytes(const PersistLayout& l) {
+    return 10 * l.n_entries + 32 * l.n_board + (l.R > kPersistRmax ? 16 * l.n_int : 0);
+}
+inline bool persist_layout_fits(const PersistLayout& l, const PersistNeeds& pn, const PersistFit& f, bool& stream) {
+    stream = pn.fixed + 10 * (size_t)pn.need > f.lds_total;
+    return 10.0 * (double)l.n_entries <= f.max_mb * 1e6 && pn.fixed <= f.lds_total && !(l.R >= 16 && !stream) && !(l.R > kPersistRmax && (f.plain || !f.wide));
+}
+struct PersistForm {
+    bool sym = false, stream = false;
+    int R = 0;
+};
+inline bool persist_form_no_worse(const PersistForm& a, const PersistForm& than) { return a.sym == than.sym && a.R <= than.R && (!a.stream || than.stream); }
+struct PersistBalance {
+    int rounds = 0;
+    PersistFit fit;
+    bool have_ref = false;
+    PersistForm ref;
+    int64_t ref_bytes = 0;
+    bool must_beat_ref = false;
+    int tried = 0, kept = 0;
+    int64_t max_bytes = 0, sum_bytes = 0;
+    int64_t max_bytes0 = 0, sum_bytes0 = 0;
+};
+inline bool persist_usable(const PersistBalance& b, const PersistLayout& l, const PersistForm& f, bool fits) {
+    if (!fits) return false;
+    if (!b.have_ref) return true;
+    return persist_form_no_worse(f, b.ref) && (!b.must_beat_ref || persist_layout_bytes(l) < b.ref_bytes);
+}
+inline bool persist_balance_wanted(const PersistBalance& b, const PersistLayout& l0, const PersistForm& f0, bool fits0) {
+    return b.rounds > 0 && l0.G >= 2 && b.sum_bytes0 > 0 && persist_usable(b, l0, f0, fits0) && b.max_bytes0 * l0.G * 100 > b.sum_bytes0 * 101;
+}
+inline bool persist_balance_keeps(const PersistBalance& b, const PersistLayout& cand, const PersistForm& fc, bool fits, int64_t cand_max, const PersistForm& held,
+                                  int64_t held_max, int64_t bytes0) {
+    return cand_max < held_max && persist_usable(b, cand, fc, fits) && persist_form_no_worse(fc, held) && persist_layout_bytes(cand) * 1000 <= bytes0 * 1005 &&
+           (!b.have_ref || (persist_layout_bytes(cand) < b.ref_bytes) == (bytes0 < b.ref_bytes));
+}
 int host_build_persist_layout_bisect(const HostSpace& hs, bool use_bnd, int G, int lds_entries, PersistLayout& pl, int sym_mode, const uint32_t* q,
-                                     std::vector<int32_t>* perm_out = nullptr, std::vector<int32_t>* rows_out = nullptr);
+                                     std::vector<int32_t>* perm_out = nullptr, std::vector<int32_t>* rows_out = nullptr, PersistBalance* bal = nullptr);
 
 }
 #endif
diff --git a/fdapde-core_amd/csrc/persist_engine.hip b/fdapde-core_amd/csrc/persist_engine.hip
--- a/fdapde-core_amd/csrc/persist_engine.hip
+++ b/fdapde-core_amd/csrc/persist_engine.hip
@@ -22,15 +22,21 @@
                                   pl.sym ? 1 : 0, balance) != FDAPDE_OK) return fail(c, FDAPDE_EHIP, "set-up check: host persistent layout failed");
     return compare_dev_persist(c, pl, dp, ref);
 }
-int check_dev_persist_bisect(fdapde_ctx* c, int v, const PersistLayout& pl, const DevPersist& dp, const std::vector<int32_t>& perm, const std::vector<int32_t>& rows) {
+int check_dev_persist_bisect(fdapde_ctx* c, int v, const PersistLayout& pl, const DevPersist& dp, const std::vector<int32_t>& perm, const std::vector<int32_t>& rows,
+                             const PersistBalance& bal) {
     if (int rc = ensure_host(c, kHostPattern | kHostDofs)) return rc;
     std::vector<uint32_t> q;
     host_bisect_quantise(c->hs.N, c->hs.n_dofs, c->hs.dof_coords.data(), c->hs.dof_i2e.data(), persist_bisect_span(c->hs.M, c->hs.N, c->hs.n_dofs), q);
     PersistLayout ref;
     ref.single_rows = pl.single_rows;
     std::vector<int32_t> perm_h, rows_h;
-    if (host_build_persist_layout_bisect(c->hs, v == 1, pl.G, 12000, ref, pl.sym ? 1 : 0, q.data(), &perm_h, &rows_h) != FDAPDE_OK)
+    PersistBalance bal_h = bal;
+    if (host_build_persist_layout_bisect(c->hs, v == 1, pl.G, 12000, ref, pl.sym ? 1 : 0, q.data(), &perm_h, &rows_h, &bal_h) != FDAPDE_OK)
         return fail(c, FDAPDE_EHIP, "set-up check: host bisection layout failed");
+    const bool same_bal = bal_h.tried == bal.tried && bal_h.kept == bal.kept && bal_h.max_bytes == bal.max_bytes && bal_h.sum_bytes == bal.sum_bytes;
+    std::fprintf(stderr, "persist check %-9s: %s (rounds tried %d / %d, kept %d / %d, largest block %lld / %lld bytes)\n", "bis_bal", same_bal ? "ok" : "MISMATCH", bal.tried,
+                 bal_h.tried, bal.kept, bal_h.kept, (long long)bal.max_bytes, (long long)bal_h.max_bytes);
+    if (!same_bal) return fail(c, FDAPDE_EHIP, "FDAPDE_SETUP_CHECK: the device builder's balance rounds differ from the host's (see stderr)");
     const bool same_perm = perm == perm_h, same_rows = rows == rows_h;
     std::fprintf(stderr, "persist check %-9s: %s (%zu elements)\n", "bis_perm", same_perm ? "ok" : "MISMATCH", perm_h.size());
     std::fprintf(stderr, "persist check %-9s: %s (%zu elements)\n", "bis_rows", same_rows ? "ok" : "MISMATCH", rows_h.size());
@@ -64,23 +70,6 @@
     }
     if (bad) return fail(c, FDAPDE_EHIP, "FDAPDE_SETUP_CHECK: the device-built persistent layout differs from the host builder's (see stderr)");
     return FDAPDE_OK;
-}
-
-struct PersistNeeds {
-    int S = 0, imp_cap = 0, exp_cap = 0;
-    size_t fixed = 0;
-    int64_t need = 0;
-};
-static PersistNeeds persist_needs(const PersistLayout& pl, bool host_built) {
-    PersistNeeds n;
-    n.S = pl.R * kPersistT;
-    n.imp_cap = (pl.max_imp + 63) & ~63, n.exp_cap = (pl.max_exp + 63) & ~63;
-    n.fixed = pl.sym ? 8 * (size_t)(n.S + n.imp_cap) + 8 * (size_t)n.S + 64 : 8 * (size_t)(n.S + n.imp_cap) + 4 * (size_t)n.imp_cap + 2 * (size_t)n.exp_cap + 64;
-    if (pl.R > kPersistRmax) n.fixed = 8 * (size_t)(n.S + n.imp_cap) + 64;
-    n.need = pl.max_block;
-    for (int g = 0; g < pl.G && host_built; ++g) n.need = std::max<int64_t>(n.need, pl.ell_off[(size_t)g + 1] - pl.ell_off[(size_t)g]);
-    n.need += 128;
-    return n;
 }
 
 int build_persist_once(fdapde_ctx* c, int v, const std::vector<int32_t>* block_rows, bool balance) {
@@ -186,6 +175,10 @@
         DevPersist dp2;
         pl2.single_rows = c->persist_single_rows;
         std::vector<int32_t> perm2, rows2;
+        PersistBalance bal;
+        bal.rounds = c->persist_balance_rounds;
+        bal.fit.lds_total = lds_total, bal.fit.max_mb = max_mb, bal.fit.plain = c->persist_plain != 0, bal.fit.wide = c->persist_wide != 0;
+        bal.have_ref = true, bal.ref.sym = pl.sym, bal.ref.R = pl.R, bal.ref.stream = ps.stream, bal.ref_bytes = persist_layout_bytes(pl), bal.must_beat_ref = part != 1;
         int rc2 = FDAPDE_EUNSUPPORTED;
         const size_t n_co = (size_t)c->hs.n_dofs * c->hs.N;
         if (on_device) {
@@ -198,19 +191,19 @@
                 coords = coords_tmp.p;
             if (coords)
                 rc2 = dev_build_persist_layout_bisect(c->hs.n_dofs, c->hs.max_row, c->rowptr.p, c->colidx.p, c->bnd.p, v == 1, c->hs.M, c->hs.N, coords, c->dof_i2e.p, pl.G, 12000,
-                                                      pl.sym ? 1 : 0, c->stream, pl2, &dp2, check ? &perm2 : nullptr, check ? &rows2 : nullptr, c->err);
+                                                      pl.sym ? 1 : 0, c->stream, pl2, &dp2, check ? &perm2 : nullptr, check ? &rows2 : nullptr, c->err, &bal);
             if (coords_tmp.p) (void)hipStreamSynchronize(c->stream);
         } else if (ensure_host(c, kHostPattern | kHostDofs) == FDAPDE_OK && c->hs.dof_coords.size() == n_co) {
             std::vector<uint32_t> q;
             host_bisect_quantise(c->hs.N, c->hs.n_dofs, c->hs.dof_coords.data(), c->hs.dof_i2e.data(), persist_bisect_span(c->hs.M, c->hs.N, c->hs.n_dofs), q);
-            rc2 = host_build_persist_layout_bisect(c->hs, v == 1, pl.G, 12000, pl2, pl.sym ? 1 : 0, q.data());
+            rc2 = host_build_persist_layout_bisect(c->hs, v == 1, pl.G, 12000, pl2, pl.sym ? 1 : 0, q.data(), nullptr, nullptr, &bal);
         }
         if (rc2 != FDAPDE_OK) {
             (void)hipGetLastError();
             c->err.clear();
         }
         if (rc2 == FDAPDE_OK && check)
-            if (int rc3 = check_dev_persist_bisect(c, v, pl2, dp2, perm2, rows2)) {
+            if (int rc3 = check_dev_persist_bisect(c, v, pl2, dp2, perm2, rows2, bal)) {
                 dev_persist_release(&dp), dev_persist_release(&dp2);
                 return rc3;
             }
@@ -219,18 +212,18 @@
         bool stream2 = false;
         if (rc2 == FDAPDE_OK) {
             pn2 = persist_needs(pl2, !on_device);
-            stream2 = pn2.fixed + 10 * (size_t)pn2.need > lds_total;
-            auto bytes = [](const PersistLayout& l) {
-                return 10.0 * (double)l.n_entries + 32.0 * (double)l.n_board + (l.R > kPersistRmax ? 16.0 * (double)l.n_int : 0.0);
-            };
-            const bool fits = 10.0 * (double)pl2.n_entries <= max_mb * 1e6 && pn2.fixed <= lds_total && !(pl2.R >= 16 && !stream2) &&
-                              !(pl2.R > kPersistRmax && (c->persist_plain || !c->persist_wide));
-            const bool same_form = pl2.sym == pl.sym && pl2.R <= pl.R && (!stream2 || ps.stream);
-            take = fits && same_form && (part == 1 || bytes(pl2) < bytes(pl));
+            auto bytes = [](const PersistLayout& l) { return (double)persist_layout_bytes(l); };
+            const bool fits = persist_layout_fits(pl2, pn2, bal.fit, stream2);
+            PersistForm f2;
+            f2.sym = pl2.sym, f2.R = pl2.R, f2.stream = stream2;
+            take = persist_usable(bal, pl2, f2, fits);
             if (std::getenv("FDAPDE_DEBUG_SETUP"))
                 std::fprintf(stderr, "persistent CG layout %d: bisection %s: %.0f bytes per iteration against %.0f (entries %lld / %lld, board %lld / %lld, imports <= %d / %d, R %d / %d)\n",
                              v, take ? "taken" : "not taken", bytes(pl2), bytes(pl), (long long)pl2.n_entries, (long long)pl.n_entries, (long long)pl2.n_board,
                              (long long)pl.n_board, pl2.max_imp, pl.max_imp, pl2.R, pl.R);
+            if (std::getenv("FDAPDE_DEBUG_SETUP"))
+                std::fprintf(stderr, "persistent CG layout %d: balance rounds tried %d, kept %d: largest block %lld -> %lld bytes per iteration (mean %lld -> %lld)\n", v, bal.tried,
+                             bal.kept, (long long)bal.max_bytes0, (long long)bal.max_bytes, (long long)(bal.sum_bytes0 / pl2.G), (long long)(bal.sum_bytes / pl2.G));
         }
         if (take) {
             dev_persist_release(&dp);
@@ -283,6 +276,21 @@
                      (long long)pl.n_int, (long long)pl.n_entries, (long long)pl.nnz,
                      100.0 * (double)(pl.n_entries - pl.nnz) / (double)(pl.n_entries > 0 ? pl.n_entries : 1), ps.lds_bytes,
                      ps.stream ? "blocks stream" : "blocks resident", pl.sym ? (pl.bisect ? ", symmetric storage, bisection blocks" : ", symmetric storage") : (pl.bisect ? ", bisection blocks" : ""), (long long)need, pl.max_imp, pl.max_exp, (long long)pl.n_board);
+    if (!pl.bisect) {
+        std::vector<int64_t> B, h_ell((size_t)pl.G + 1);
+        std::vector<int32_t> h_exp((size_t)pl.G + 1), h_imp((size_t)pl.G + 1);
+        if (on_device) {
+            HIPCHK(c, hipMemcpy(h_ell.data(), ps.ell_off.p, sizeof(int64_t) * h_ell.size(), hipMemcpyDeviceToHost));
+            HIPCHK(c, hipMemcpy(h_exp.data(), ps.exp_off.p, sizeof(int32_t) * h_exp.size(), hipMemcpyDeviceToHost));
+            HIPCHK(c, hipMemcpy(h_imp.data(), ps.imp_off.p, sizeof(int32_t) * h_imp.size(), hipMemcpyDeviceToHost));
+        } else
+            h_ell = pl.ell_off, h_exp = pl.exp_off, h_imp = pl.imp_off;
+        pl.bal_kept = 0;
+        persist_block_bytes(pl.G, h_ell.data(), h_exp.data(), h_imp.data(), B, pl.bal_max, pl.bal_sum);
+    }
+    if (std::getenv("FDAPDE_DEBUG_SETUP"))
+        std::fprintf(stderr, "persistent CG layout %d: balance rounds kept %d, largest block %lld bytes per iteration, mean %lld\n", v, pl.bal_kept, (long long)pl.bal_max,
+                     (long long)(pl.bal_sum / pl.G));
     pl.slot_dof = {}, pl.ell_code = {}, pl.ell_src = {}, pl.exp_slot = {}, pl.imp_pos = {}, pl.sl_off = {}, pl.ell_off = {};
     ps.meta = std::move(pl);
     ps.filled = false, ps.ok = true;
diff --git a/include/fdapde_hip.h b/include/fdapde_hip.h
--- a/include/fdapde_hip.h
+++ b/include/fdapde_hip.h
@@ -126,6 +126,8 @@
 int fdapde_solver_layout_kind(fdapde_ctx *ctx, int32_t with_dirichlet, int32_t *kind, int32_t *symmetric_storage,
                               int32_t *workgroups, int32_t *rows_per_thread);
 int fdapde_solver_layout_partition(fdapde_ctx *ctx, int32_t with_dirichlet, int32_t *partition);
+int fdapde_solver_layout_balance(fdapde_ctx *ctx, int32_t with_dirichlet, int32_t *rounds_kept, int64_t *max_block_bytes,
+                                 int64_t *mean_block_bytes);
 typedef int (*fdapde_allreduce_fn)(void *user, double *host_buf, int64_t count);
 int fdapde_comm_init_callback(fdapde_ctx *ctx, int32_t world, int32_t rank, fdapde_allreduce_fn fn, void *user);
 int fdapde_comm_unique_id(void *out128);
```
